# imedslab/OAProgressionMMF

Measured on AMD Instinct MI355X. Metric: knees/sec full XR+MRI+clin fusion train step, higher is better.
Workload: dtype f32; 1 GPU; syn3: XR1MR3C1CnnTrf train step (fwd+FocalLoss+bwd+Adam), per-GPU batch 8, global batch 8, BASELINE config 4 on BASELINE's synthetic tensors: XR 1x310x310 + 3 x MRI 1x160x384x384 (slice-major) + 9 clinical; random-init weights; parallelism=dp1, activation_recompute=012,012,01

## Files before the change

### include/koaf.h

```cpp
#ifndef KOAF_H
#define KOAF_H
#include <stdint.h>
#ifdef __cplusplus
extern "C" {
#endif

#define KOAF_OK 0
#define KOAF_EINVAL (-1)
#define KOAF_ELAUNCH (-2)

int koaf_version(void);
const char* koaf_last_error(void);
int koaf_set_status_buffer(uint32_t* dev4);

typedef struct KoafOperand {
    const float* ptr;
    int64_t ld;
    int64_t bs0, bs1;
    int64_t tap_stride;
    int64_t tap_stride_h;
    int32_t kind;
    int32_t gather;
    int32_t H, W, C;
    int32_t CS;
    int32_t PH, PW;
    int32_t KH, KW, stride, pad;
    int32_t pad_w;
    int32_t _pad1;
    int32_t tf;
    int32_t tf_bs;
    const float* sc;
    const float* sh;
    const uint16_t* planes;
    int64_t plane_stride;
    const float* amax;
    float fscale;
    int32_t _pad4;
    const float* ptr2;
    const float* sc2;
    const uint16_t* zeros;
    float* side;
    const float* sh2;
} KoafOperand;

typedef struct KoafGemm {
    KoafOperand A, B;
    int32_t M, N, K;
    int32_t nb0, nb1;
    int32_t splitk;
    int32_t bm, bn;
    float* C;
    int64_t ldc, cbs0, cbs1;
    float alpha;
    int32_t prec;
    const float* bias;
    const float* residual;
    int64_t ldr, rbs0, rbs1;
    float* stats;
    int64_t stats_ld;
    int64_t stats_bs;
    int32_t cmap, cm_PH, cm_PW, cm_H, cm_W, cm_py, cm_px, _pad2;
    int32_t bnb_mode;
    int32_t fmt;
    const float* bnb_c;
    const float* bnb_y;
    const float* bnb_sc;
    const float* bnb_sh;
    const float* bnb_mean;
    const float* bnb_invstd;
    const float* bnb2_c;
    const float* bnb2_mean;
    const float* bnb2_invstd;
    float* bnb_part;
    float* bnb_amax;
    int32_t m_base, part_row0;
    const float* stats_shift;
    uint32_t* status;
    int32_t act16;
    int32_t _pad5;
    uint16_t* out_planes;
    const float* out_sc;
    const float* out_sh;
    int64_t out_ps;
} KoafGemm;

int koaf_gemm(const KoafGemm* g, void* stream);
int koaf_gemm_pick_tile(const KoafGemm* g, int32_t* bm, int32_t* bn);
int koaf_gemm_part_rows(const KoafGemm* g);
typedef struct KoafLaunchRec {
    char variant[24];
    int32_t bm, bn;
    int32_t tiles, grid_x;
    int32_t splitk, nbatch;
    int32_t fmt, a_tf, b_tf, act16;
    int32_t M, N, K;
    int32_t emit;
} KoafLaunchRec;
int koaf_launch_log(int on);
int koaf_launch_log_read(KoafLaunchRec* out, int32_t cap);
int koaf_slab_reduce(const float* slabs, int32_t nslab, int64_t n, float* out, void* stream);
int koaf_slab_reduce_epilogue(const float* slabs, int32_t nslab, int32_t M, int32_t N, const float* bias,
                              const float* residual, int64_t ldr, float* out, int64_t ldo, void* stream);

typedef struct KoafWPlane {
    int64_t src_off, f_off, d_off, tile0;
    int32_t R, taps, C, Kp, Rp, _pad;
} KoafWPlane;
int koaf_wplanes_build(const float* base, uint16_t* planes, float* amax, const KoafWPlane* table_dev, int32_t n,
                       int64_t ntiles, void* stream);
int koaf_set_conv3x3_halo(int on);
int koaf_set_stream(int on);
int64_t koaf_act_planes_elems(int64_t npix, int32_t C);
int koaf_act_planes(const float* x, const float* x2, int64_t npix, int32_t C, int32_t tf, const float* sc, const float* sh,
                    const float* sc2, const float* amax, float fscale, uint16_t* planes, int32_t act16, void* stream);
typedef struct KoafWImg {
    const uint16_t* f;
    const uint16_t* d;
    const float* amax;
} KoafWImg;
typedef struct KoafBnApply {
    const float* dz;
    const float* c;
    const float* coef;
    const float* amax;
} KoafBnApply;


#define KOAF_ACT_SCALE 16.0f
typedef struct KoafTail {
    const float* idt;
    float* y_out;
    const float* idt_sc;
    const float* idt_sh;
} KoafTail;
typedef struct KoafEmit {
    uint16_t* planes;
    const float* sc;
    const float* sh;
} KoafEmit;
int koaf_conv2d_fwd(const float* x, const float* w, float* y, int32_t N, int32_t H, int32_t W,
                    int32_t Cin, int32_t Cout, int32_t KH, int32_t KW, int32_t stride, int32_t pad,
                    const float* in_sc, const float* in_sh, float* stats, int32_t* stats_rows,
                    const float* stats_shift, const KoafWImg* wimg, const uint16_t* x_planes, const KoafTail* tail,
                    const KoafEmit* emit, int32_t act16, void* stream);
int32_t koaf_conv2d_stats_rows(int64_t M, int32_t Cout);
int koaf_conv2d_dgrad(const float* dy, const float* w, float* dx, int32_t N, int32_t H, int32_t W,
                      int32_t Cin, int32_t Cout, int32_t KH, int32_t KW, int32_t stride,
                      int32_t pad, const float* residual, const KoafWImg* wimg, const float* dy_amax,
                      const KoafBnApply* dy_apply, const uint16_t* dy_planes, int32_t act16, void* stream);
typedef struct KoafBnb {
    int32_t mode, _pad;
    float* dz_amax;
    const float* c;
    const float* y;
    const float* sc;
    const float* sh;
    const float* mean;
    const float* invstd;
    const float* c2;
    const float* mean2;
    const float* invstd2;
} KoafBnb;
int32_t koaf_conv2d_dgrad_bnb_rows(int32_t N, int32_t H, int32_t W, int32_t Cin, int32_t stride);
int koaf_conv2d_dgrad_bnb(const float* dy, const float* w, float* dx, int32_t N, int32_t H, int32_t W,
                          int32_t Cin, int32_t Cout, int32_t KH, int32_t KW, int32_t stride, int32_t pad,
                          const float* residual, const KoafBnb* bnb, float* part, int32_t* part_rows,
                          const KoafWImg* wimg, const float* dy_amax, const KoafBnApply* dy_apply,
                          const uint16_t* dy_planes, int32_t act16, void* stream);
int64_t koaf_conv2d_wgrad_ws(int32_t N, int32_t H, int32_t W, int32_t Cin, int32_t Cout,
                             int32_t KH, int32_t KW, int32_t stride, int32_t pad);
int koaf_conv2d_wgrad(const float* dy, const float* x, float* dw, int32_t N, int32_t H, int32_t W,
                      int32_t Cin, int32_t Cout, int32_t KH, int32_t KW, int32_t stride,
                      int32_t pad, const float* in_sc, const float* in_sh, float* slabs,
                      const float* dy_amax, const KoafBnApply* dy_apply, const uint16_t* dy_planes,
                      const uint16_t* x_planes, int32_t act16, void* stream);

int koaf_gconv_expand_w(const float* w, float* wexp, int32_t C, int32_t groups, float* amax, void* stream);
int koaf_gconv_compress_dw(const float* dwexp, float* dw, int32_t C, int32_t groups, void* stream);
int koaf_gconv3x3_fwd(const float* x, const float* wexp, float* y, int32_t N, int32_t H, int32_t W,
                      int32_t C, int32_t stride, const float* in_sc, const float* in_sh,
                      float* stats, int32_t* stats_rows, const float* stats_shift, const float* w_amax, int32_t act16, void* stream);
int koaf_gconv3x3_dgrad(const float* dy, const float* wexp, float* dx, int32_t N, int32_t H,
                        int32_t W, int32_t C, int32_t stride, const float* w_amax, const float* dy_amax, void* stream);
int64_t koaf_gconv3x3_wgrad_ws(int32_t N, int32_t H, int32_t W, int32_t C, int32_t stride);
int koaf_gconv3x3_wgrad(const float* dy, const float* x, float* dwexp, int32_t N, int32_t H,
                        int32_t W, int32_t C, int32_t stride, const float* in_sc,
                        const float* in_sh, float* slabs, const float* dy_amax, int32_t act16, void* stream);

int32_t koaf_stem_stats_rows(int32_t N, int32_t H);
int koaf_stem_fwd(const float* x, const float* w1t, float* y, int32_t N, int32_t H, int32_t W,
                  float* stats, const float* stats_shift, int32_t act16, void* stream);
int64_t koaf_stem_wgrad_ws(int32_t N, int32_t H, int32_t W);
int koaf_stem_wgrad(const float* dy, const float* x, float* dw1t, int32_t N, int32_t H, int32_t W,
                    float* slabs, const KoafBnApply* dy_apply, int32_t act16, void* stream);
int koaf_stem_fold_w(const float* w, float* w1t, void* stream);
int koaf_stem_unfold_dw(const float* dw1t, float* dw, void* stream);

int koaf_colstats(const float* x, int64_t rows, int32_t C, float* part, int32_t* part_rows,
                  const float* shift, int32_t act16, void* stream);
int32_t koaf_colpart_rows(int64_t rows, int32_t C);
int64_t koaf_bn_reduce_ws(int32_t rows, int32_t C);
int koaf_bn_finalize(const float* stats, int32_t rows, int32_t C, int64_t count,
                     const float* gamma, const float* beta, float* running_mean,
                     float* running_var, int64_t* num_batches_tracked, float momentum, float eps,
                     int32_t train, float* mean, float* invstd, float* sc, float* sh,
                     const float* shift, double* ws, void* stream);
int koaf_bn_add_relu(const float* c, const float* sc, const float* sh, const float* idt,
                     const float* idsc, const float* idsh, float* y, int64_t rows, int32_t C,
                     int32_t act16, void* stream);
int koaf_bn_relu(const float* c, const float* sc, const float* sh, float* y, int64_t rows,
                 int32_t C, int32_t act16, void* stream);
int koaf_bn_bwd_reduce(const float* g, const float* c, const float* ymask, const float* sc,
                       const float* sh, const float* mean, const float* invstd, int32_t mask_mode,
                       float* dz_out, float* part, int32_t* part_rows, int64_t rows, int32_t C,
                       float* dz_amax, int32_t act16, void* stream);
int koaf_bn_bwd_reduce_pool(const float* pool_g, const uint8_t* pool_argmax, const float* c, const float* sc,
                            const float* sh, const float* mean, const float* invstd, float* dz_out, float* part,
                            int32_t* part_rows, int32_t N, int32_t H, int32_t W, int32_t C, float* dz_amax,
                            int32_t act16, void* stream);
int koaf_bn_bwd_finalize(const float* part, int32_t part_rows, int32_t C, int64_t count,
                         const float* sc, const float* invstd, float* dgamma, float* dbeta,
                         float* coef, int32_t nsum, int32_t i1, double* ws, const float* mean,
                         const float* dz_amax, float* amax, void* stream);
int koaf_bn_bwd_apply(const float* dz, const float* c, const float* mean, const float* coef,
                      float* dc, int64_t rows, int32_t C, float* amax, int32_t act16, void* stream);

int koaf_widen(const void* x, int32_t dtype, float* y, int64_t n, void* stream);
int64_t koaf_minmax_ws(int64_t n);
int koaf_minmax(const float* x, int32_t B, int64_t n, float* mm, float* ws, void* stream);
int koaf_augment(const float* x, float* y, const float* mm, const float* params, int32_t B, int32_t R, int32_t C,
                 int32_t S, float mean, float stdv, void* stream);

int koaf_maxpool_fwd(const float* c, const float* sc, const float* sh, float* y, uint8_t* argmax,
                     int32_t N, int32_t H, int32_t W, int32_t C, int32_t act16, void* stream);
int koaf_maxpool_bwd(const float* dy, const uint8_t* argmax, float* da, int32_t N, int32_t H,
                     int32_t W, int32_t C, void* stream);
int koaf_gap_fwd(const float* y, float* out, int32_t N, int32_t HW, int32_t C, int32_t act16, void* stream);
int koaf_gap_bwd(const float* dout, float* dy, int32_t N, int32_t HW, int32_t C, void* stream);

int koaf_slice_fold(const float* x, float* out, int32_t B, int32_t R, int32_t Cc, int32_t S,
                    void* stream);
int koaf_downscale2(const float* x, float* out, int32_t B, int32_t R, int32_t Cc, int32_t S,
                    int32_t fs, void* stream);

int koaf_resize(const float* x, float* out, int64_t BC, int32_t ndim, const int32_t* in_size, const int32_t* out_size,
                void* stream);

int64_t koaf_linear_ws(int32_t M, int32_t N, int32_t K);
int koaf_linear_fwd(const float* x, const float* w, const float* b, const float* residual,
                    float* y, float* ws, int32_t M, int32_t N, int32_t K, void* stream);
int koaf_linear_dgrad(const float* dy, const float* w, const float* residual, float* dx, float* ws,
                      int32_t M, int32_t N, int32_t K, void* stream);
int koaf_linear_wgrad(const float* dy, const float* x, float* dw, float* db, float* ws, int32_t M,
                      int32_t N, int32_t K, void* stream);
int koaf_layernorm_fwd(const float* x, const float* gamma, const float* beta, float* y,
                       float* mean, float* rstd, int32_t rows, int32_t D, float eps, void* stream);
int64_t koaf_layernorm_bwd_ws(int32_t rows, int32_t D);
int koaf_layernorm_bwd(const float* dy, const float* x, const float* gamma, const float* mean,
                       const float* rstd, float* dx, float* dgamma, float* dbeta, float* part,
                       int32_t rows, int32_t D, void* stream);
int koaf_attention_fwd(const float* qkv, float* attn, float* out, int32_t B, int32_t n, int32_t h,
                       int32_t d, float scale, void* stream);
int koaf_attention_bwd(const float* dout, const float* qkv, const float* attn, float* dqkv,
                       float* ws, int32_t B, int32_t n, int32_t h, int32_t d, float scale,
                       void* stream);
int koaf_softmax_rows(float* x, int64_t rows, int32_t n, void* stream);
int koaf_softmax_bwd_rows(float* dp, const float* p, int64_t rows, int32_t n, float scale,
                          void* stream);
int koaf_gelu_fwd(const float* x, float* y, int64_t n, void* stream);
int koaf_gelu_bwd(const float* dy, const float* x, float* dx, int64_t n, void* stream);
int koaf_relu_fwd(const float* x, float* y, int64_t n, void* stream);
int koaf_relu_bwd(const float* dy, const float* y, float* dx, int64_t n, void* stream);
int koaf_dropout(const float* x, float* y, int64_t n, float p, uint64_t seed, const int64_t* epoch, void* stream);
int koaf_counter_add(int64_t* counter, int64_t delta, void* stream);
int koaf_dropout2d(const float* x, float* y, int32_t N, int32_t HW, int32_t C, float p, uint64_t seed,
                   const int64_t* epoch, void* stream);
int koaf_add(const float* a, const float* b, float* out, int64_t n, void* stream);
int64_t koaf_colsum_ws(int32_t rows, int32_t C);
int koaf_colsum(const float* x, float* out, int32_t rows, int32_t C, float* part, void* stream);

int64_t koaf_loss_ws(int32_t B, int64_t S);
int koaf_focal_loss(const float* logits, const int64_t* target, const float* class_weight, float* loss, float* dlogits,
                    int32_t B, int32_t C, int64_t S, float gamma, int32_t reduction_mean, float* ws, void* stream);
int koaf_ce_loss(const float* logits, const int64_t* target, const float* class_weight, float* loss, float* dlogits,
                 int32_t B, int32_t C, int64_t S, float* ws, void* stream);

int koaf_adam_step(float* p, const float* g, float* m, float* v, int64_t n, float lr, double beta1,
                   double beta2, float eps, float weight_decay, int32_t step, int32_t adamw,
                   const float* hyper, float* vmax, void* stream);
int koaf_adam_hyper(int32_t* step, const float* lr, double beta1, double beta2, float* hyper, void* stream);
int koaf_fill(float* p, float value, int64_t n, void* stream);

#ifdef __cplusplus
}
#endif
#endif
```

### oaprogressionmmf_amd/_lib.py

```python
import ctypes
import os
import re
from pathlib import Path

_ROOT = Path(__file__).resolve().parent
HEADER = _ROOT.parent / "include" / "koaf.h"
LIB_PATH = _ROOT / "csrc" / "libkoaf.so"


class KoafOperand(ctypes.Structure):
    _fields_ = [
        ("ptr", ctypes.c_void_p),
        ("ld", ctypes.c_int64),
        ("bs0", ctypes.c_int64),
        ("bs1", ctypes.c_int64),
        ("tap_stride", ctypes.c_int64),
        ("tap_stride_h", ctypes.c_int64),
        ("kind", ctypes.c_int32),
        ("gather", ctypes.c_int32),
        ("H", ctypes.c_int32),
        ("W", ctypes.c_int32),
        ("C", ctypes.c_int32),
        ("CS", ctypes.c_int32),
        ("PH", ctypes.c_int32),
        ("PW", ctypes.c_int32),
        ("KH", ctypes.c_int32),
        ("KW", ctypes.c_int32),
        ("stride", ctypes.c_int32),
        ("pad", ctypes.c_int32),
        ("pad_w", ctypes.c_int32),
        ("_pad1", ctypes.c_int32),
        ("tf", ctypes.c_int32),
        ("tf_bs", ctypes.c_int32),
        ("sc", ctypes.c_void_p),
        ("sh", ctypes.c_void_p),
        ("planes", ctypes.c_void_p),
        ("plane_stride", ctypes.c_int64),
        ("amax", ctypes.c_void_p),
        ("fscale", ctypes.c_float),
        ("_pad4", ctypes.c_int32),
        ("ptr2", ctypes.c_void_p),
        ("sc2", ctypes.c_void_p),
        ("zeros", ctypes.c_void_p),
        ("side", ctypes.c_void_p),
        ("sh2", ctypes.c_void_p),
    ]


class KoafGemm(ctypes.Structure):
    _fields_ = [
        ("A", KoafOperand),
        ("B", KoafOperand),
        ("M", ctypes.c_int32),
        ("N", ctypes.c_int32),
        ("K", ctypes.c_int32),
        ("nb0", ctypes.c_int32),
        ("nb1", ctypes.c_int32),
        ("splitk", ctypes.c_int32),
        ("bm", ctypes.c_int32),
        ("bn", ctypes.c_int32),
        ("C", ctypes.c_void_p),
        ("ldc", ctypes.c_int64),
        ("cbs0", ctypes.c_int64),
        ("cbs1", ctypes.c_int64),
        ("alpha", ctypes.c_float),
        ("prec", ctypes.c_int32),
        ("bias", ctypes.c_void_p),
        ("residual", ctypes.c_void_p),
        ("ldr", ctypes.c_int64),
        ("rbs0", ctypes.c_int64),
        ("rbs1", ctypes.c_int64),
        ("stats", ctypes.c_void_p),
        ("stats_ld", ctypes.c_int64),
        ("stats_bs", ctypes.c_int64),
        ("cmap", ctypes.c_int32),
        ("cm_PH", ctypes.c_int32),
        ("cm_PW", ctypes.c_int32),
        ("cm_H", ctypes.c_int32),
        ("cm_W", ctypes.c_int32),
        ("cm_py", ctypes.c_int32),
        ("cm_px", ctypes.c_int32),
        ("_pad2", ctypes.c_int32),
        ("bnb_mode", ctypes.c_int32),
        ("fmt", ctypes.c_int32),
        ("bnb_c", ctypes.c_void_p),
        ("bnb_y", ctypes.c_void_p),
        ("bnb_sc", ctypes.c_void_p),
        ("bnb_sh", ctypes.c_void_p),
        ("bnb_mean", ctypes.c_void_p),
        ("bnb_invstd", ctypes.c_void_p),
        ("bnb2_c", ctypes.c_void_p),
        ("bnb2_mean", ctypes.c_void_p),
        ("bnb2_invstd", ctypes.c_void_p),
        ("bnb_part", ctypes.c_void_p),
        ("bnb_amax", ctypes.c_void_p),
        ("m_base", ctypes.c_int32),
        ("part_row0", ctypes.c_int32),
        ("stats_shift", ctypes.c_void_p),
        ("status", ctypes.c_void_p),
        ("act16", ctypes.c_int32),
        ("_pad5", ctypes.c_int32),
        ("out_planes", ctypes.c_void_p),
        ("out_sc", ctypes.c_void_p),
        ("out_sh", ctypes.c_void_p),
        ("out_ps", ctypes.c_int64),
    ]


class KoafBnb(ctypes.Structure):
    _fields_ = [
        ("mode", ctypes.c_int32),
        ("_pad", ctypes.c_int32),
        ("dz_amax", ctypes.c_void_p),
        ("c", ctypes.c_void_p),
        ("y", ctypes.c_void_p),
        ("sc", ctypes.c_void_p),
        ("sh", ctypes.c_void_p),
        ("mean", ctypes.c_void_p),
        ("invstd", ctypes.c_void_p),
        ("c2", ctypes.c_void_p),
        ("mean2", ctypes.c_void_p),
        ("invstd2", ctypes.c_void_p),
    ]


class KoafWPlane(ctypes.Structure):
    _fields_ = [
        ("src_off", ctypes.c_int64),
        ("f_off", ctypes.c_int64),
        ("d_off", ctypes.c_int64),
        ("tile0", ctypes.c_int64),
        ("R", ctypes.c_int32),
        ("taps", ctypes.c_int32),
        ("C", ctypes.c_int32),
        ("Kp", ctypes.c_int32),
        ("Rp", ctypes.c_int32),
        ("_pad", ctypes.c_int32),
    ]


class KoafWImg(ctypes.Structure):
    _fields_ = [("f", ctypes.c_void_p), ("d", ctypes.c_void_p), ("amax", ctypes.c_void_p)]


class KoafTail(ctypes.Structure):
    _fields_ = [("idt", ctypes.c_void_p), ("y_out", ctypes.c_void_p), ("idt_sc", ctypes.c_void_p), ("idt_sh", ctypes.c_void_p)]


class KoafEmit(ctypes.Structure):
    _fields_ = [("planes", ctypes.c_void_p), ("sc", ctypes.c_void_p), ("sh", ctypes.c_void_p)]


class KoafBnApply(ctypes.Structure):
    _fields_ = [("dz", ctypes.c_void_p), ("c", ctypes.c_void_p), ("coef", ctypes.c_void_p), ("amax", ctypes.c_void_p)]


class KoafLaunchRec(ctypes.Structure):
    _fields_ = [
        ("variant", ctypes.c_char * 24),
        ("bm", ctypes.c_int32),
        ("bn", ctypes.c_int32),
        ("tiles", ctypes.c_int32),
        ("grid_x", ctypes.c_int32),
        ("splitk", ctypes.c_int32),
        ("nbatch", ctypes.c_int32),
        ("fmt", ctypes.c_int32),
        ("a_tf", ctypes.c_int32),
        ("b_tf", ctypes.c_int32),
        ("act16", ctypes.c_int32),
        ("M", ctypes.c_int32),
        ("N", ctypes.c_int32),
        ("K", ctypes.c_int32),
        ("emit", ctypes.c_int32),
    ]


_SCALARS = {
    "int": ctypes.c_int,
    "int32_t": ctypes.c_int32,
    "int64_t": ctypes.c_int64,
    "uint64_t": ctypes.c_uint64,
    "uint32_t": ctypes.c_uint32,
    "float": ctypes.c_float,
    "double": ctypes.c_double,
}


def _ctype(decl: str):
    decl = decl.strip()
    if "*" in decl:
        base = decl.replace("const", "").replace("*", "").split()[0]
        if base == "KoafGemm":
            return ctypes.POINTER(KoafGemm)
        if base == "KoafBnb":
            return ctypes.POINTER(KoafBnb)
        if base == "KoafWImg":
            return ctypes.POINTER(KoafWImg)
        if base == "KoafBnApply":
            return ctypes.POINTER(KoafBnApply)
        if base == "KoafTail":
            return ctypes.POINTER(KoafTail)
        if base == "KoafEmit":
            return ctypes.POINTER(KoafEmit)
        if base == "KoafLaunchRec":
            return ctypes.POINTER(KoafLaunchRec)
        if base == "char":
            return ctypes.c_char_p
        return ctypes.c_void_p
    toks = decl.replace("const", "").split()
    return _SCALARS[toks[0]]


def parse_header(path=HEADER):
    text = Path(path).read_text()
    text = re.sub(r"/\*.*?\*/", " ", text, flags=re.S)
    text = re.sub(r"typedef struct.*?\}\s*\w+;", " ", text, flags=re.S)
    text = re.sub(r"^\s*#.*$", " ", text, flags=re.M)
    protos = {}
    for m in re.finditer(r"([\w\s\*]+?)\b(koaf_\w+)\s*\(([^)]*)\)\s*;", text):
        ret, name, args = m.group(1).strip(), m.group(2), m.group(3).strip()
        if args in ("void", ""):
            argtypes = []
        else:
            argtypes = []
            for a in args.split(","):
                a = a.strip()
                mm = re.match(r"(.*?)(\w+)$", a)
                argtypes.append(_ctype(mm.group(1) if mm.group(1).strip() else a))
        protos[name] = (_ctype(ret) if ret != "void" else None, argtypes)
    return protos


_LIB = None


class KoafError(RuntimeError):
    pass


def lib():
    global _LIB
    if _LIB is not None:
        return _LIB
    path = Path(os.environ.get("KOAF_LIB", LIB_PATH))
    if not path.exists():
        raise KoafError(
            f"libkoaf.so not found at {path}: build it with `python -c 'import __graft_entry__ as g; "
            f"g.build()'` or `make -C oaprogressionmmf_amd/csrc` -- there is no CPU fallback")
    handle = ctypes.CDLL(str(path))
    for name, (restype, argtypes) in parse_header().items():
        fn = getattr(handle, name)
        fn.restype = restype
        fn.argtypes = argtypes
    _LIB = handle
    return _LIB


def check(rc, what=""):
    if rc != 0:
        msg = lib().koaf_last_error()
        raise KoafError(f"{what}: rc={rc}: {msg.decode() if msg else '?'}")
```

### oaprogressionmmf_amd/csrc/koaf_common.h

```cpp
#pragma once
#include <hip/hip_runtime.h>
#include <stdint.h>
#include <stdio.h>
#include "../../include/koaf.h"

typedef float v4f __attribute__((ext_vector_type(4)));
typedef float v16f __attribute__((ext_vector_type(16)));
typedef int v4i __attribute__((ext_vector_type(4)));
typedef long long v4l __attribute__((ext_vector_type(4)));

void koaf_set_error(const char* fmt, ...);

#define KOAF_REQUIRE(cond, ...)            \
    do {                                   \
        if (!(cond)) {                     \
            koaf_set_error(__VA_ARGS__);   \
            return KOAF_EINVAL;            \
        }                                  \
    } while (0)

static inline int koaf_check_launch(const char* what) {
    hipError_t e = hipGetLastError();
    if (e != hipSuccess) {
        koaf_set_error("%s: launch failed: %s", what, hipGetErrorString(e));
        return KOAF_ELAUNCH;
    }
    return KOAF_OK;
}

static inline int64_t cdiv64(int64_t a, int64_t b) { return (a + b - 1) / b; }
static inline bool aligned16(const void* p) { return (((uintptr_t)p) & 15) == 0; }

__device__ __forceinline__ float wave_sum(float v) {
#pragma unroll
    for (int o = 32; o > 0; o >>= 1) v += __shfl_xor(v, o, 64);
    return v;
}
__device__ __forceinline__ float wave_max(float v) {
#pragma unroll
    for (int o = 32; o > 0; o >>= 1) v = fmaxf(v, __shfl_xor(v, o, 64));
    return v;
}

__device__ __forceinline__ unsigned koaf_absbits(float x) { return __float_as_uint(x) & 0x7fffffffu; }
__device__ __forceinline__ bool koaf_bits_finite(unsigned absbits) { return absbits < 0x7f800000u; }
__device__ __forceinline__ unsigned wave_max_u(unsigned v) {
#pragma unroll
    for (int o = 32; o > 0; o >>= 1) { const unsigned w = (unsigned)__shfl_xor((int)v, o, 64); v = v > w ? v : w; }
    return v;
}

__device__ __forceinline__ void block_amax_raise_bits(unsigned bits, float* slot) {
    __shared__ unsigned koaf_amax_red[16];
    bits = wave_max_u(bits);
    const int w = threadIdx.x >> 6, nw = (blockDim.x + 63) >> 6;
    if ((threadIdx.x & 63) == 0) koaf_amax_red[w] = bits;
    __syncthreads();
    if (threadIdx.x == 0) {
        unsigned m = koaf_amax_red[0];
        for (int i = 1; i < nw; ++i) m = m > koaf_amax_red[i] ? m : koaf_amax_red[i];
        if (m > __hip_atomic_load(reinterpret_cast<unsigned*>(slot), __ATOMIC_RELAXED, __HIP_MEMORY_SCOPE_AGENT))
            atomicMax(reinterpret_cast<unsigned*>(slot), m);
    }
}
__device__ __forceinline__ void block_amax_raise(float v, float* slot) { block_amax_raise_bits(koaf_absbits(v), slot); }

uint32_t* koaf_status_ptr();
__device__ __forceinline__ void koaf_status_add(uint32_t* st, int slot, unsigned n) {
    if (st != nullptr && n != 0u) atomicAdd(&st[slot], n);
}

typedef __bf16 koaf_bf16x2 __attribute__((ext_vector_type(2)));
__device__ __forceinline__ v4f widen_bf16x4(unsigned lo, unsigned hi) {
    return (v4f){__uint_as_float(lo << 16), __uint_as_float(lo & 0xffff0000u), __uint_as_float(hi << 16), __uint_as_float(hi & 0xffff0000u)};
}
__device__ __forceinline__ uint2 round_bf16x4(v4f v) {
    typedef float v2f_ __attribute__((ext_vector_type(2)));
    const unsigned a = __builtin_bit_cast(unsigned, __builtin_convertvector((v2f_){v[0], v[1]}, koaf_bf16x2));
    const unsigned b = __builtin_bit_cast(unsigned, __builtin_convertvector((v2f_){v[2], v[3]}, koaf_bf16x2));
    return make_uint2(a, b);
}
template <bool H>
__device__ __forceinline__ v4f load4_nt(const float* p, int64_t off) {
    if constexpr (!H) return __builtin_nontemporal_load((const v4f*)(p + off));
    else {
        const unsigned short* q = reinterpret_cast<const unsigned short*>(p) + off;
        const unsigned lo = __builtin_nontemporal_load((const unsigned*)q), hi = __builtin_nontemporal_load((const unsigned*)q + 1);
        return widen_bf16x4(lo, hi);
    }
}
template <bool H>
__device__ __forceinline__ void store4_nt(float* p, int64_t off, v4f v) {
    if constexpr (!H) __builtin_nontemporal_store(v, (v4f*)(p + off));
    else {
        const uint2 u = round_bf16x4(v);
        unsigned* q = (unsigned*)(reinterpret_cast<unsigned short*>(p) + off);
        __builtin_nontemporal_store(u.x, q);
        __builtin_nontemporal_store(u.y, q + 1);
    }
}

template <bool H>
__device__ __forceinline__ v4f load4(const float* p, int64_t off) {
    if constexpr (!H) return *(const v4f*)(p + off);
    else {
        const uint2 u = *(const uint2*)(reinterpret_cast<const unsigned short*>(p) + off);
        return widen_bf16x4(u.x, u.y);
    }
}
template <bool H>
__device__ __forceinline__ void store4(float* p, int64_t off, v4f v) {
    if constexpr (!H) *(v4f*)(p + off) = v;
    else *(uint2*)(reinterpret_cast<unsigned short*>(p) + off) = round_bf16x4(v);
}
```

### oaprogressionmmf_amd/csrc/koaf_conv.hip

```cpp
#include <string.h>
#include "koaf_common.h"
#include <stdlib.h>

namespace {

inline void zero_gemm(KoafGemm* g) { *g = KoafGemm{}; g->alpha = 1.f; g->nb0 = g->nb1 = 1; g->splitk = 1; }

inline int conv_out(int H, int K, int s, int p) { return (H + 2 * p - K) / s + 1; }

inline int64_t rup32(int64_t v) { return (v + 31) / 32 * 32; }

inline void set_fimg(KoafGemm* g, const KoafWImg* w, int R, int64_t K) {
    g->fmt = 1;
    g->A.fscale = KOAF_ACT_SCALE;
    g->B.amax = w->amax;
    if (!w->f) return;
    g->B.kind = 2; g->B.gather = 0;
    g->B.planes = w->f; g->B.ld = rup32(K); g->B.plane_stride = (int64_t)R * g->B.ld;
}

inline void set_aplanes(KoafOperand* a, const uint16_t* planes, int64_t plane_elems) {
    a->kind = 2; a->planes = planes; a->plane_stride = plane_elems; a->zeros = planes + 2 * plane_elems;
    a->ptr = nullptr; a->ptr2 = nullptr; a->tf = 0; a->sc = a->sh = a->sc2 = nullptr;
}
// ... 95 lines not shown
            if (oy < OH) {
                if (ox < OW) put((((int64_t)n * OH + oy) * OW + ox) * 64 + co, a0);
                if (ox + 1 < OW) put((((int64_t)n * OH + oy) * OW + ox + 1) * 64 + co, a1);
            }
        }
    }
    if constexpr (ST) {
        __shared__ float sred[2][ST_TH][64];
        sred[0][pg][co] = s1;
        sred[1][pg][co] = s2;
        __syncthreads();
        if (pg < 2) {
            float a = 0.f;
#pragma unroll
            for (int g = 0; g < ST_TH; ++g) a += sred[pg][g][co];
            part[((int64_t)blockIdx.x * 2 + pg) * 64 + co] = a;
        }
    }
}

template <bool APPLY, bool C16>
__global__ void __launch_bounds__(256) stem_wgrad_kernel(const float* __restrict__ dy, const float* __restrict__ x,
                                                         float* __restrict__ slabs, int N, int H, int W, int OH,
                                                         int OW, const float* __restrict__ cc, const float* __restrict__ coef) {
    __shared__ __attribute__((aligned(16))) float patch[ST_PH][ST_PW];
    __shared__ float red[3][64][49 + 1];
    const int co = threadIdx.x & 63, pg = threadIdx.x >> 6;
    const int tx = (OW + ST_TW - 1) / ST_TW, ty = (OH + ST_TH - 1) / ST_TH;
    const int ntile = N * ty * tx;
    float acc[49];
#pragma unroll
    for (int k = 0; k < 49; ++k) acc[k] = 0.f;
    float k0 = 1.f, k2 = 0.f, k3 = 0.f;
    if constexpr (APPLY) { k0 = coef[co]; k2 = coef[128 + co]; k3 = coef[192 + co]; }
    auto grad = [&](int64_t o) {
        float gv = dy[o];
        if constexpr (APPLY) {
            float cv;
            if constexpr (C16) cv = __uint_as_float((unsigned)reinterpret_cast<const unsigned short*>(cc)[o] << 16);
            else cv = cc[o];
            gv = fmaf(k0, gv, fmaf(-k2, cv, k3));
        }
        return gv;
    };
    for (int tile = blockIdx.x; tile < ntile; tile += gridDim.x) {
        int b = tile;
        const int bx = b % tx; b /= tx;
        const int by = b % ty;
        const int n = b / ty;
        const int oy0 = by * ST_TH, ox0 = bx * ST_TW;
        __syncthreads();
        stem_load_patch(patch, x, n, H, W, oy0, ox0);
        __syncthreads();
        const int oy = oy0 + pg;
#pragma unroll 1
        for (int q = 0; q < ST_TW / 2; ++q) {
            const int ox = ox0 + 2 * q;
            float g0 = 0.f, g1 = 0.f;
            if (oy < OH) {
                if (ox < OW) g0 = grad((((int64_t)n * OH + oy) * OW + ox) * 64 + co);
                if (ox + 1 < OW) g1 = grad((((int64_t)n * OH + oy) * OW + ox + 1) * 64 + co);
            }
#pragma unroll
            for (int kh = 0; kh < 7; ++kh) {
                const float* pr = &patch[2 * pg + kh][4 * q];
                const v4f p0 = *(const v4f*)pr, p1 = *(const v4f*)(pr + 4);
                const float p8 = pr[8];
                const float pv[9] = {p0[0], p0[1], p0[2], p0[3], p1[0], p1[1], p1[2], p1[3], p8};
#pragma unroll
                for (int kw = 0; kw < 7; ++kw) acc[kh * 7 + kw] += g0 * pv[kw] + g1 * pv[kw + 2];
            }
        }
    }
    __syncthreads();
    if (pg > 0) {
#pragma unroll
        for (int k = 0; k < 49; ++k) red[pg - 1][co][k] = acc[k];
    }
    __syncthreads();
    if (pg == 0) {
        float* sl = slabs + (int64_t)blockIdx.x * 49 * 64;
#pragma unroll
        for (int k = 0; k < 49; ++k) sl[k * 64 + co] = acc[k] + red[0][co][k] + red[1][co][k] + red[2][co][k];
    }
}

__global__ void stem_fold_kernel(const float* __restrict__ w, float* __restrict__ w1t) {
    const int i = blockIdx.x * blockDim.x + threadIdx.x;
    if (i >= 64 * 49) return;
    const int co = i / 49, k = i - co * 49;
    const float* s = w + (int64_t)i * 3;
    w1t[k * 64 + co] = s[0] + s[1] + s[2];
}
__global__ void stem_unfold_kernel(const float* __restrict__ dw1t, float* __restrict__ dw) {
    const int i = blockIdx.x * blockDim.x + threadIdx.x;
    if (i >= 64 * 49) return;
    const int co = i / 49, k = i - co * 49;
    const float v = dw1t[k * 64 + co];
    dw[(int64_t)i * 3 + 0] = v;
    dw[(int64_t)i * 3 + 1] = v;
    dw[(int64_t)i * 3 + 2] = v;
}

__global__ void __launch_bounds__(256) gconv_expand_kernel(const float* __restrict__ w, float* __restrict__ wexp,
                                                           int C, int Cg, float* __restrict__ amax) {
    const int64_t total = (int64_t)C * 9 * 64;
    unsigned mb = 0u;
    for (int64_t i = (int64_t)blockIdx.x * 256 + threadIdx.x; i < total; i += (int64_t)gridDim.x * 256) {
        const int ci = (int)(i & 63);
        int64_t r = i >> 6;
        const int tap = (int)(r % 9);
        const int co = (int)(r / 9);
        const int col = co & 63;
        const int g0 = (col / Cg) * Cg;
        float v = 0.f;
        if (ci >= g0 && ci < g0 + Cg) v = w[((int64_t)co * 9 + tap) * Cg + (ci - g0)];
        wexp[i] = v;
        mb = max(mb, koaf_absbits(v));
    }
    if (amax != nullptr) block_amax_raise_bits(mb, amax);
}
__global__ void __launch_bounds__(256) gconv_compress_kernel(const float* __restrict__ dwexp, float* __restrict__ dw,
                                                             int C, int Cg) {
    const int64_t total = (int64_t)C * 9 * Cg;
    for (int64_t i = (int64_t)blockIdx.x * 256 + threadIdx.x; i < total; i += (int64_t)gridDim.x * 256) {
        const int cg = (int)(i % Cg);
        int64_t r = i / Cg;
        const int tap = (int)(r % 9);
        const int co = (int)(r / 9);
        const int g0 = ((co & 63) / Cg) * Cg;
        dw[i] = dwexp[((int64_t)co * 9 + tap) * 64 + g0 + cg];
    }
}

}

#define STREAM ((hipStream_t)stream)

extern "C" int koaf_conv2d_fwd(const float* x, const float* w, float* y, int32_t N, int32_t H, int32_t W, int32_t Cin,
                               int32_t Cout, int32_t KH, int32_t KW, int32_t stride, int32_t pad, const float* in_sc,
                               const float* in_sh, float* stats, int32_t* stats_rows, const float* stats_shift,
                               const KoafWImg* wimg, const uint16_t* x_planes, const KoafTail* tail, const KoafEmit* emit,
                               int32_t act16, void* stream) {
    KOAF_REQUIRE((x || x_planes) && w && y && N > 0 && Cin % 32 == 0 && Cout % 4 == 0, "koaf_conv2d_fwd: bad args (Cin=%d Cout=%d)",
                 Cin, Cout);
    KOAF_REQUIRE(!tail || (tail->idt && x && in_sc && in_sh && !x_planes && KH == 1 && KW == 1 && stride == 1 && pad == 0 && wimg &&
                           wimg->amax && wimg->f && (tail->idt_sc == nullptr) == (tail->idt_sh == nullptr)),
                 "koaf_conv2d_fwd: the fused bottleneck tail serves 1x1 / stride-1 convolutions with weight plane images, from x / in_sc / in_sh");
    KOAF_REQUIRE((in_sc == nullptr) == (in_sh == nullptr), "koaf_conv2d_fwd: in_sc/in_sh come together");
    const int OH = conv_out(H, KH, stride, pad), OW = conv_out(W, KW, stride, pad);
    const int64_t M = (int64_t)N * OH * OW;
    KOAF_REQUIRE(M < (1ll << 31), "koaf_conv2d_fwd: too many output pixels");
    KoafGemm g;
    zero_gemm(&g);
    g.A.ptr = x;
    g.A.kind = 0;
    if (KH == 1 && KW == 1 && stride == 1 && pad == 0 && !x_planes) {
        g.A.gather = 0;
        g.A.ld = Cin;
    } else {
        g.A.gather = 1;
        g.A.H = H; g.A.W = W; g.A.C = Cin; g.A.CS = Cin;
        g.A.PH = OH; g.A.PW = OW;
        g.A.KH = KH; g.A.KW = KW; g.A.stride = stride; g.A.pad = pad; g.A.pad_w = pad;
    }
    if (in_sc) { g.A.tf = 1; g.A.sc = in_sc; g.A.sh = in_sh; }
    if (tail) { g.A.tf = 3; g.A.ptr2 = tail->idt; g.A.side = tail->y_out; g.A.sc2 = tail->idt_sc; g.A.sh2 = tail->idt_sc ? tail->idt_sh : nullptr; }
    g.B.ptr = w;
    g.B.kind = 0;
    g.B.ld = (int64_t)KH * KW * Cin;
    g.M = (int)M; g.N = Cout; g.K = KH * KW * Cin;
    if (wimg && wimg->amax) set_fimg(&g, wimg, Cout, g.K);
    if (x_planes) {
        KOAF_REQUIRE(g.A.gather == 1 && g.B.kind == 2, "koaf_conv2d_fwd: x_planes serve the gathered kernels and need wimg->f");
        set_aplanes(&g.A, x_planes, (int64_t)N * H * W * Cin);
    }
    g.C = y; g.ldc = Cout;
    g.stats = stats;
    g.stats_shift = stats ? stats_shift : nullptr;
    g.act16 = act16 ? 1 : 0;
    if (emit) {
        KOAF_REQUIRE(emit->planes && emit->sc && emit->sh && (Cout % 8) == 0, "koaf_conv2d_fwd: emit needs planes / sc / sh and Cout %% 8 == 0");
        g.out_planes = emit->planes; g.out_sc = emit->sc; g.out_sh = emit->sh; g.out_ps = M * Cout;
    }
    if (stats_rows) *stats_rows = koaf_gemm_part_rows(&g);
    return koaf_gemm(&g, stream);
}

extern "C" int32_t koaf_conv2d_stats_rows(int64_t M, int32_t Cout) { return (int32_t)cdiv64(M, 64); }

static void set_apply(KoafOperand* a, const KoafBnApply* ap, int C) {
    a->ptr = ap->dz; a->ptr2 = ap->c; a->tf = 2;
    a->sc = ap->coef; a->sc2 = ap->coef + 2 * (int64_t)C; a->sh = ap->coef + 3 * (int64_t)C;
    a->amax = ap->amax;
}

static void set_bnb(KoafGemm* g, const KoafBnb* b, float* part) {
    if (!b) return;
    g->bnb_amax = b->dz_amax;
    g->bnb_mode = b->mode;
    g->bnb_c = b->c; g->bnb_y = b->y; g->bnb_sc = b->sc; g->bnb_sh = b->sh;
    g->bnb_mean = b->mean; g->bnb_invstd = b->invstd;
    g->bnb2_c = b->c2; g->bnb2_mean = b->mean2; g->bnb2_invstd = b->invstd2;
    g->bnb_part = part;
}

extern "C" int32_t koaf_conv2d_dgrad_bnb_rows(int32_t N, int32_t H, int32_t W, int32_t Cin, int32_t stride) {
    if (stride == 2) {
        int64_t r = 0;
        for (int py = 0; py < 2; ++py)
            for (int px = 0; px < 2; ++px) r += cdiv64((int64_t)N * ((H - py + 1) / 2) * ((W - px + 1) / 2), 64);
        return (int32_t)r;
    }
    return (int32_t)cdiv64((int64_t)N * H * W, 64);
}

extern "C" int koaf_conv2d_dgrad_bnb(const float* dy, const float* w, float* dx, int32_t N, int32_t H, int32_t W,
                                     int32_t Cin, int32_t Cout, int32_t KH, int32_t KW, int32_t stride, int32_t pad,
                                     const float* residual, const KoafBnb* bnb, float* part, int32_t* part_rows,
                                     const KoafWImg* wimg, const float* dy_amax, const KoafBnApply* dy_apply,
                                     const uint16_t* dy_planes, int32_t act16, void* stream) {
    KOAF_REQUIRE(!dy_planes || (wimg && wimg->amax && wimg->d && (dy_amax || dy_apply) && KH * KW > 1),
                 "koaf_conv2d_dgrad: dy_planes need the weight's D plane image, dy_amax and a gathered (KH*KW > 1) kernel");
    KOAF_REQUIRE((dy || dy_apply || dy_planes) && w && dx && N > 0 && Cout % 32 == 0 && Cin % 4 == 0, "koaf_conv2d_dgrad: bad args");
    KOAF_REQUIRE(!dy_apply || (dy_apply->dz && dy_apply->c && dy_apply->coef && dy_apply->amax && wimg && wimg->amax && wimg->d),
                 "koaf_conv2d_dgrad: dy_apply needs dz / c / coef / amax and the weight's D plane image");
    if (dy_apply) { dy = dy_apply->dz; dy_amax = dy_apply->amax; }
    if (bnb && bnb->dz_amax && hipMemsetAsync(bnb->dz_amax, 0, sizeof(float), (hipStream_t)stream) != hipSuccess) {
        koaf_set_error("koaf_conv2d_dgrad_bnb: memset failed");
        return KOAF_ELAUNCH;
    }
    const bool f16 = wimg && wimg->amax && dy_amax;
    const bool ps = f16 && wimg->d != nullptr;
    const uint16_t* w_dimg = ps ? wimg->d : nullptr;
    const int64_t dld = (int64_t)KH * KW * Cout, dps = (int64_t)Cin * dld;
    KOAF_REQUIRE(!bnb || (part && part_rows), "koaf_conv2d_dgrad_bnb: part / part_rows required");
    const int nsum = (bnb && bnb->c2) ? 3 : 2;
    int rows_done = 0;
    const int OH = conv_out(H, KH, stride, pad), OW = conv_out(W, KW, stride, pad);
    const int64_t M = (int64_t)N * H * W;
    KOAF_REQUIRE(M < (1ll << 31), "koaf_conv2d_dgrad: too many pixels");
    KoafGemm g;
    if (stride == 2) {
        for (int py = 0; py < 2; ++py)
            for (int px = 0; px < 2; ++px) {
                const int Hc = (H - py + 1) / 2, Wc = (W - px + 1) / 2;
                if (Hc <= 0 || Wc <= 0) continue;
                const int khs = (py + pad) & 1, kws = (px + pad) & 1;
                const int nkh = khs < KH ? (KH - khs + 1) / 2 : 0, nkw = kws < KW ? (KW - kws + 1) / 2 : 0;
                const int offy = (py + pad - khs) / 2, offx = (px + pad - kws) / 2;
                zero_gemm(&g);
                g.prec = 1;
                if (f16) { g.fmt = 1; g.A.amax = dy_amax; g.B.amax = wimg->amax; }
                g.A.ptr = dy; g.A.kind = 0; g.A.gather = 2;
                if (dy_apply) set_apply(&g.A, dy_apply, Cout);
                g.A.H = OH; g.A.W = OW; g.A.C = Cout; g.A.CS = Cout;
                g.A.PH = Hc; g.A.PW = Wc;
                g.A.KH = nkh > 0 ? nkh : 1; g.A.KW = nkw > 0 ? nkw : 1; g.A.stride = 1; g.A.pad = offy; g.A.pad_w = offx;
                g.B.ptr = w + ((int64_t)khs * KW + kws) * Cin; g.B.kind = 1; g.B.gather = 3;
                g.B.C = Cout; g.B.ld = (int64_t)KH * KW * Cin;
                g.B.KW = g.A.KW; g.B.tap_stride = 2ll * Cin; g.B.tap_stride_h = 2ll * KW * Cin;
                if (ps) {
                    g.B.kind = 2; g.B.gather = 0;
                    g.B.planes = w_dimg + ((int64_t)khs * KW + kws) * Cout; g.B.ld = dld; g.B.plane_stride = dps;
                    g.B.tap_stride = 2ll * Cout; g.B.tap_stride_h = 2ll * KW * Cout;
                }
                if (dy_planes && nkh > 0 && nkw > 0) set_aplanes(&g.A, dy_planes, (int64_t)N * OH * OW * Cout);
                g.M = N * Hc * Wc; g.N = Cin; g.K = nkh * nkw * Cout;
                g.C = dx; g.ldc = Cin;
                g.residual = residual; g.ldr = Cin;
                g.cmap = 1; g.cm_PH = Hc; g.cm_PW = Wc; g.cm_H = H; g.cm_W = W; g.cm_py = py; g.cm_px = px;
                if (bnb) {
                    set_bnb(&g, bnb, part + (int64_t)rows_done * nsum * Cin);
                    rows_done += koaf_gemm_part_rows(&g);
                }
                g.act16 = act16 ? 2 : 0;
                int rc = koaf_gemm(&g, stream);
                if (rc != KOAF_OK) return rc;
            }
        if (part_rows) *part_rows = rows_done;
        return KOAF_OK;
    }
    zero_gemm(&g);
    g.prec = 1;
    if (f16) { g.fmt = 1; g.A.amax = dy_amax; g.B.amax = wimg->amax; }
    g.A.ptr = dy;
    g.A.kind = 0;
    if (dy_apply) set_apply(&g.A, dy_apply, Cout);
    g.B.ptr = w;
    g.B.kind = 1;
    if (KH == 1 && KW == 1 && stride == 1 && pad == 0) {
        g.A.gather = 0;
        g.A.ld = Cout;
        g.B.gather = 0;
        g.B.ld = Cin;
    } else {
        g.A.gather = 2;
        g.A.H = OH; g.A.W = OW; g.A.C = Cout; g.A.CS = Cout;
        g.A.PH = H; g.A.PW = W;
        g.A.KH = KH; g.A.KW = KW; g.A.stride = stride; g.A.pad = pad; g.A.pad_w = pad;
        g.B.gather = 3;
        g.B.C = Cout;
        g.B.ld = (int64_t)KH * KW * Cin;
        g.B.KW = KW;
        g.B.tap_stride = Cin;
        g.B.tap_stride_h = (int64_t)KW * Cin;
    }
    if (ps) {
        g.B.kind = 2; g.B.gather = 0; g.B.C = 0; g.B.tap_stride = g.B.tap_stride_h = 0;
        g.B.planes = w_dimg; g.B.ld = dld; g.B.plane_stride = dps;
    }
    if (dy_planes) set_aplanes(&g.A, dy_planes, (int64_t)N * OH * OW * Cout);
    g.M = (int)M; g.N = Cin; g.K = KH * KW * Cout;
    g.C = dx; g.ldc = Cin;
    g.residual = residual; g.ldr = Cin;
    if (bnb) {
        set_bnb(&g, bnb, part);
        *part_rows = koaf_gemm_part_rows(&g);
    }
    g.act16 = act16 ? 2 : 0;
    return koaf_gemm(&g, stream);
}

extern "C" int koaf_conv2d_dgrad(const float* dy, const float* w, float* dx, int32_t N, int32_t H, int32_t W,
                                 int32_t Cin, int32_t Cout, int32_t KH, int32_t KW, int32_t stride, int32_t pad,
                                 const float* residual, const KoafWImg* wimg, const float* dy_amax,
                                 const KoafBnApply* dy_apply, const uint16_t* dy_planes, int32_t act16, void* stream) {
    return koaf_conv2d_dgrad_bnb(dy, w, dx, N, H, W, Cin, Cout, KH, KW, stride, pad, residual, nullptr, nullptr,
                                 nullptr, wimg, dy_amax, dy_apply, dy_planes, act16, stream);
}

bool koaf_wgrad3_ring_ok(int N, int H, int W, int Cin, int Cout);
int64_t koaf_wgrad3_ring_ws(int N, int H, int W, int Cin, int Cout);
int koaf_wgrad3_ring(const uint16_t* dy_planes, const uint16_t* x_planes, float* dw, float* slabs, const float* dy_amax,
                     float x_scale, int N, int H, int W, int Cin, int Cout, void* stream);
static inline bool wgrad3_ring_shape(int N, int H, int W, int Cin, int Cout, int KH, int KW, int stride, int pad) {
    return KH == 3 && KW == 3 && stride == 1 && pad == 1 && koaf_wgrad3_ring_ok(N, H, W, Cin, Cout);
}

extern "C" int64_t koaf_conv2d_wgrad_ws(int32_t N, int32_t H, int32_t W, int32_t Cin, int32_t Cout, int32_t KH,
                                        int32_t KW, int32_t stride, int32_t pad) {
    const int OH = conv_out(H, KH, stride, pad), OW = conv_out(W, KW, stride, pad);
    WgradPlan p = wgrad_plan(Cout, KH * KW * Cin, (int64_t)N * OH * OW, Cin, 1);
    int64_t ws = p.splitk > 1 ? (int64_t)(p.splitk + 16) * Cout * KH * KW * Cin : 0;
    if (wgrad3_ring_shape(N, H, W, Cin, Cout, KH, KW, stride, pad)) {
        const int64_t w3 = koaf_wgrad3_ring_ws(N, H, W, Cin, Cout);
        if (w3 > ws) ws = w3;
    }
    return ws;
}

extern "C" int koaf_conv2d_wgrad(const float* dy, const float* x, float* dw, int32_t N, int32_t H, int32_t W,
                                 int32_t Cin, int32_t Cout, int32_t KH, int32_t KW, int32_t stride, int32_t pad,
                                 const float* in_sc, const float* in_sh, float* slabs, const float* dy_amax,
                                 const KoafBnApply* dy_apply, const uint16_t* dy_planes, const uint16_t* x_planes,
                                 int32_t act16, void* stream) {
    KOAF_REQUIRE((dy_planes == nullptr) == (x_planes == nullptr) && (!dy_planes || dy_amax || dy_apply),
                 "koaf_conv2d_wgrad: dy_planes and x_planes come together, with dy_amax (or dy_apply)");
    KOAF_REQUIRE((dy || dy_apply || dy_planes) && (x || x_planes) && dw && N > 0 && Cin % 64 == 0 && Cout % 4 == 0, "koaf_conv2d_wgrad: bad args");
    KOAF_REQUIRE(!dy_apply || (dy_apply->dz && dy_apply->c && dy_apply->coef && dy_apply->amax),
                 "koaf_conv2d_wgrad: dy_apply needs dz / c / coef / amax");
    if (dy_apply) { dy = dy_apply->dz; dy_amax = dy_apply->amax; }
    KOAF_REQUIRE((in_sc == nullptr) == (in_sh == nullptr), "koaf_conv2d_wgrad: in_sc/in_sh come together");
    const int OH = conv_out(H, KH, stride, pad), OW = conv_out(W, KW, stride, pad);
    const int64_t P = (int64_t)N * OH * OW;
    KOAF_REQUIRE(P < (1ll << 31), "koaf_conv2d_wgrad: too many pixels");
    const int Ntot = KH * KW * Cin;
    if (dy_planes && slabs && wgrad3_ring_shape(N, H, W, Cin, Cout, KH, KW, stride, pad))
        return koaf_wgrad3_ring(dy_planes, x_planes, dw, slabs, dy_amax, KOAF_ACT_SCALE, N, H, W, Cin, Cout, stream);
    WgradPlan p = wgrad_plan(Cout, Ntot, P, Cin, 1);
    KOAF_REQUIRE(p.splitk == 1 || slabs, "koaf_conv2d_wgrad: workspace required");
    KoafGemm g;
    zero_gemm(&g);
    g.prec = 1;
    if (dy_amax) { g.fmt = 1; g.A.amax = dy_amax; g.B.fscale = KOAF_ACT_SCALE; }
    g.A.ptr = dy; g.A.kind = 1; g.A.ld = Cout;
    if (dy_apply) set_apply(&g.A, dy_apply, Cout);
    g.B.ptr = x; g.B.kind = 1;
    if (KH == 1 && KW == 1 && stride == 1 && pad == 0) {
        g.B.gather = 0;
        g.B.ld = Cin;
    } else {
        g.B.gather = 1;
        g.B.H = H; g.B.W = W; g.B.C = Cin; g.B.CS = Cin;
        g.B.PH = OH; g.B.PW = OW;
        g.B.KH = KH; g.B.KW = KW; g.B.stride = stride; g.B.pad = pad; g.B.pad_w = pad;
    }
    if (in_sc) { g.B.tf = 1; g.B.sc = in_sc; g.B.sh = in_sh; }
    if (dy_planes) {
        set_aplanes(&g.A, dy_planes, P * Cout);
        g.A.kind = 3; g.A.ld = Cout;
        set_aplanes(&g.B, x_planes, (int64_t)N * H * W * Cin);
        g.B.kind = 3; g.B.gather = 1;
        g.B.H = H; g.B.W = W; g.B.C = Cin; g.B.CS = Cin;
        g.B.PH = OH; g.B.PW = OW;
        g.B.KH = KH; g.B.KW = KW; g.B.stride = stride; g.B.pad = pad; g.B.pad_w = pad;
    }
    g.M = Cout; g.N = Ntot; g.K = (int)P;
    g.bm = p.bm; g.bn = p.bn; g.splitk = p.splitk;
    g.C = p.splitk > 1 ? slabs : dw;
    g.ldc = Ntot;
    g.act16 = (act16 && !dy_planes) ? 3 : 0;
    int rc = koaf_gemm(&g, stream);
    if (rc != KOAF_OK || p.splitk == 1) return rc;
    return koaf_slab_reduce(slabs, p.splitk, (int64_t)Cout * Ntot, dw, stream);
}

extern "C" int koaf_gconv_expand_w(const float* w, float* wexp, int32_t C, int32_t groups, float* amax, void* stream) {
    KOAF_REQUIRE(w && wexp && C % 64 == 0 && groups > 0 && C % groups == 0 && 64 % (C / groups) == 0,
                 "koaf_gconv_expand_w: C=%d groups=%d unsupported", C, groups);
    hipLaunchKernelGGL(gconv_expand_kernel, dim3(1024), dim3(256), 0, STREAM, w, wexp, C, C / groups, amax);
    return koaf_check_launch("koaf_gconv_expand_w");
}
extern "C" int koaf_gconv_compress_dw(const float* dwexp, float* dw, int32_t C, int32_t groups, void* stream) {
    KOAF_REQUIRE(dwexp && dw && C % 64 == 0 && groups > 0 && C % groups == 0 && 64 % (C / groups) == 0,
                 "koaf_gconv_compress_dw: C=%d groups=%d unsupported", C, groups);
    hipLaunchKernelGGL(gconv_compress_kernel, dim3(512), dim3(256), 0, STREAM, dwexp, dw, C, C / groups);
    return koaf_check_launch("koaf_gconv_compress_dw");
}

extern "C" int koaf_gconv3x3_fwd(const float* x, const float* wexp, float* y, int32_t N, int32_t H, int32_t W,
                                 int32_t C, int32_t stride, const float* in_sc, const float* in_sh, float* stats,
                                 int32_t* stats_rows, const float* stats_shift, const float* w_amax, int32_t act16, void* stream) {
    KOAF_REQUIRE(x && wexp && y && N > 0 && C % 64 == 0, "koaf_gconv3x3_fwd: bad args");
    const int OH = conv_out(H, 3, stride, 1), OW = conv_out(W, 3, stride, 1);
    const int64_t M = (int64_t)N * OH * OW;
    KOAF_REQUIRE(M < (1ll << 31), "koaf_gconv3x3_fwd: too many pixels");
    KoafGemm g;
    zero_gemm(&g);
    g.nb1 = C / 64;
    g.A.ptr = x; g.A.kind = 0; g.A.gather = 1; g.A.bs1 = 64;
    g.A.H = H; g.A.W = W; g.A.C = 64; g.A.CS = C; g.A.PH = OH; g.A.PW = OW;
    g.A.KH = 3; g.A.KW = 3; g.A.stride = stride; g.A.pad = 1; g.A.pad_w = 1;
    if (in_sc) { g.A.tf = 1; g.A.sc = in_sc; g.A.sh = in_sh; }
    g.B.ptr = wexp; g.B.kind = 0; g.B.ld = 576; g.B.bs1 = 64 * 576;
    g.M = (int)M; g.N = 64; g.K = 576;
    g.C = y; g.ldc = C; g.cbs1 = 64;
    g.stats = stats; g.stats_ld = C; g.stats_bs = 64;
    g.stats_shift = stats ? stats_shift : nullptr;
    g.bn = 64; g.bm = 128;
    if (stats_rows) *stats_rows = (int)cdiv64(M, g.bm);
    g.A.tf_bs = 64;
    g.act16 = act16 ? 1 : 0;
    if (w_amax && !act16) { g.fmt = 1; g.A.fscale = KOAF_ACT_SCALE; g.B.amax = w_amax; }
    return koaf_gemm(&g, stream);
}

extern "C" int koaf_gconv3x3_dgrad(const float* dy, const float* wexp, float* dx, int32_t N, int32_t H, int32_t W,
                                   int32_t C, int32_t stride, const float* w_amax, const float* dy_amax, void* stream) {
    KOAF_REQUIRE(dy && wexp && dx && N > 0 && C % 64 == 0, "koaf_gconv3x3_dgrad: bad args");
    const int OH = conv_out(H, 3, stride, 1), OW = conv_out(W, 3, stride, 1);
    const int64_t M = (int64_t)N * H * W;
    KOAF_REQUIRE(M < (1ll << 31), "koaf_gconv3x3_dgrad: too many pixels");
    KoafGemm g;
    zero_gemm(&g);
    g.prec = 1;
    g.nb1 = C / 64;
    g.A.ptr = dy; g.A.kind = 0; g.A.gather = 2; g.A.bs1 = 64;
    g.A.H = OH; g.A.W = OW; g.A.C = 64; g.A.CS = C; g.A.PH = H; g.A.PW = W;
    g.A.KH = 3; g.A.KW = 3; g.A.stride = stride; g.A.pad = 1; g.A.pad_w = 1;
    g.B.ptr = wexp; g.B.kind = 1; g.B.gather = 3; g.B.C = 64; g.B.ld = 576; g.B.tap_stride = 64;
    g.B.tap_stride_h = 3 * 64; g.B.KW = 3;
    g.B.bs1 = 64 * 576;
    g.M = (int)M; g.N = 64; g.K = 576;
    g.C = dx; g.ldc = C; g.cbs1 = 64;
    g.bn = 64; g.bm = 128;
    if (w_amax && dy_amax) { g.fmt = 1; g.A.amax = dy_amax; g.B.amax = w_amax; }
    return koaf_gemm(&g, stream);
}

extern "C" int64_t koaf_gconv3x3_wgrad_ws(int32_t N, int32_t H, int32_t W, int32_t C, int32_t stride) {
    const int OH = conv_out(H, 3, stride, 1), OW = conv_out(W, 3, stride, 1);
    WgradPlan p = wgrad_plan(64, 576, (int64_t)N * OH * OW, 64, C / 64);
    return (int64_t)p.splitk * C * 576;
}

extern "C" int koaf_gconv3x3_wgrad(const float* dy, const float* x, float* dwexp, int32_t N, int32_t H, int32_t W,
                                   int32_t C, int32_t stride, const float* in_sc, const float* in_sh, float* slabs,
                                   const float* dy_amax, int32_t act16, void* stream) {
    KOAF_REQUIRE(dy && x && dwexp && slabs && N > 0 && C % 64 == 0, "koaf_gconv3x3_wgrad: bad args");
    const int OH = conv_out(H, 3, stride, 1), OW = conv_out(W, 3, stride, 1);
    const int64_t P = (int64_t)N * OH * OW;
// ... 304 lines not shown
```

### oaprogressionmmf_amd/csrc/koaf_elem.hip

```cpp
#include <stdarg.h>
#include "koaf_common.h"
#include <stdlib.h>

static thread_local char g_err[512] = "";
void koaf_set_error(const char* fmt, ...) {
    va_list ap;
    va_start(ap, fmt);
    vsnprintf(g_err, sizeof(g_err), fmt, ap);
    va_end(ap);
}
extern "C" const char* koaf_last_error(void) { return g_err; }
static uint32_t* g_status = nullptr;
uint32_t* koaf_status_ptr() { return g_status; }
extern "C" int koaf_set_status_buffer(uint32_t* dev4) { g_status = dev4; return KOAF_OK; }
extern "C" int koaf_version(void) { return 190; }

namespace {

constexpr int EB = 256;

inline int ew_blocks_per_cu() {
    static const int v = [] { const char* e = getenv("KOAF_EW_BLOCKS_PER_CU"); int n = e ? atoi(e) : 32; return n < 1 ? 1 : n; }();
    return v;
}
inline unsigned ew_grid(int64_t nvec) {
    int64_t b = cdiv64(nvec, EB);
    if (b > 256 * ew_blocks_per_cu()) b = 256 * ew_blocks_per_cu();
    if (b < 1) b = 1;
    return (unsigned)b;
}

struct ColGeom {
    int CW;
    int nchunk;
    int CV;
    int RP;
    int rpb;
    int nblk;
};
inline bool col_geom(int64_t rows, int C, int max_blk, ColGeom* g) {
    if (C % 4) return false;
    int CW = C > 1024 ? 1024 : C;
    if (C % CW) return false;
    int CV = CW / 4;
    if (256 % CV) return false;
    g->CW = CW;
    g->nchunk = C / CW;
    g->CV = CV;
    g->RP = 256 / CV;
    int64_t rpb = cdiv64(rows, max_blk);
    rpb = cdiv64(rpb, g->RP) * g->RP;
    if (rpb < g->RP * 4) rpb = g->RP * 4;
    g->rpb = (int)rpb;
    g->nblk = (int)cdiv64(rows, rpb);
    return true;
}

template <int NS>
__device__ __forceinline__ void col_block_reduce(v4f (&s)[NS], float* part, int blk, int C, int c0, int CV,
                                                 int RP) {
    __shared__ v4f red[256];
    const int t = threadIdx.x;
    const int cvx = t % CV, ry = t / CV;
#pragma unroll
    for (int k = 0; k < NS; ++k) {
        __syncthreads();
        red[t] = s[k];
        __syncthreads();
        if (ry == 0) {
            v4f a = red[cvx];
            for (int j = 1; j < RP; ++j) a += red[j * CV + cvx];
            *(v4f*)&part[((int64_t)blk * NS + k) * C + c0 + 4 * cvx] = a;
        }
    }
}

template <bool H>
__global__ void __launch_bounds__(256) colstats_kernel(const float* __restrict__ x, int64_t rows, int C,
                                                       ColGeom g, float* __restrict__ part, int sq,
                                                       const float* __restrict__ shift) {
    const int t = threadIdx.x, cvx = t % g.CV, ry = t / g.CV;
    const int c0 = blockIdx.y * g.CW;
    const int64_t rbeg = (int64_t)blockIdx.x * g.rpb;
    const int64_t rend = min(rows, rbeg + (int64_t)g.rpb);
    v4f s[2] = {{0, 0, 0, 0}, {0, 0, 0, 0}};
    v4f k = {0, 0, 0, 0};
    if (shift) k = *(const v4f*)&shift[c0 + 4 * cvx];
    for (int64_t r = rbeg + ry; r < rend; r += g.RP) {
        v4f v = load4<H>(x, r * C + c0 + 4 * cvx) - k;
        s[0] += v;
        s[1] += v * v;
    }
    if (sq) col_block_reduce<2>(s, part, blockIdx.x, C, c0, g.CV, g.RP);
    else {
        v4f s1[1] = {s[0]};
        col_block_reduce<1>(s1, part, blockIdx.x, C, c0, g.CV, g.RP);
    }
}

__global__ void colsum_small_kernel(const float* __restrict__ x, int rows, int C, float* __restrict__ out) {
    int c = blockIdx.x * blockDim.x + threadIdx.x;
    if (c >= C) return;
    float a = 0.f;
    for (int r = 0; r < rows; ++r) a += x[(int64_t)r * C + c];
    out[c] = a;
}

template <int NS>
__global__ void __launch_bounds__(1024) colfinal_kernel(const float* __restrict__ part, int rows, int C,
                                                        float* __restrict__ out0, float* __restrict__ out1) {
    __shared__ double red[NS][16][64];
    const int cx = threadIdx.x & 63, gy = threadIdx.x >> 6;
    const int c = blockIdx.x * 64 + cx;
    double a[NS];
#pragma unroll
    for (int k = 0; k < NS; ++k) a[k] = 0.0;
    if (c < C)
        for (int r = gy; r < rows; r += 16)
#pragma unroll
            for (int k = 0; k < NS; ++k) a[k] += (double)part[((int64_t)r * NS + k) * C + c];
#pragma unroll
    for (int k = 0; k < NS; ++k) red[k][gy][cx] = a[k];
    __syncthreads();
    if (gy == 0 && c < C) {
#pragma unroll
        for (int k = 0; k < NS; ++k) {
            double s = 0.0;
            for (int j = 0; j < 16; ++j) s += red[k][j][cx];
            (k == 0 ? out0 : out1)[c] = (float)s;
        }
    }
}

__global__ void __launch_bounds__(1024) part_reduce_kernel(const float* __restrict__ src, int rows, int C, int nsum,
                                                           int i1, int chunk, double* __restrict__ ws) {
    __shared__ double red[2][16][64];
    const int cx = threadIdx.x & 63, gy = threadIdx.x >> 6;
    const int c = blockIdx.x * 64 + cx;
    const int r0 = blockIdx.y * chunk, r1 = min(rows, r0 + chunk);
    double a = 0.0, b = 0.0;
    if (c < C)
        for (int r = r0 + gy; r < r1; r += 16) {
            a += (double)src[((int64_t)r * nsum + 0) * C + c];
            b += (double)src[((int64_t)r * nsum + i1) * C + c];
        }
    red[0][gy][cx] = a;
    red[1][gy][cx] = b;
    __syncthreads();
    if (gy < 2 && c < C) {
        double t = 0.0;
        for (int j = 0; j < 16; ++j) t += red[gy][j][cx];
        ws[((int64_t)blockIdx.y * 2 + gy) * C + c] = t;
    }
}

static inline int part_slices(int rows) { return rows > 128 ? (rows >= 4096 ? 64 : (rows + 63) / 64) : 0; }

template <typename T>
__global__ void __launch_bounds__(1024) bn_finalize_kernel(const T* __restrict__ stats, int rows, int C,
                                                           double inv_count, double unbias,
                                                           const float* __restrict__ gamma,
                                                           const float* __restrict__ beta, float* running_mean,
                                                           float* running_var, int64_t* nbt, float momentum,
                                                           float eps, int train, float* mean, float* invstd,
                                                           float* sc, float* sh, const float* __restrict__ shift,
                                                           uint32_t* status) {
    __shared__ double red[2][16][64];
    const int cx = threadIdx.x & 63, gy = threadIdx.x >> 6;
// ... 1283 lines not shown
```

### oaprogressionmmf_amd/csrc/koaf_gemm.hip

```cpp
#include "koaf_gemm_launch.h"
#include <stdlib.h>
#include <string.h>
#include <atomic>
#include <mutex>
#include <vector>

namespace {

__global__ void __launch_bounds__(256) slab_reduce_epi_kernel(const float* __restrict__ slabs, int nslab, int M, int N,
                                                              const float* __restrict__ bias,
                                                              const float* __restrict__ residual, int64_t ldr,
                                                              float* __restrict__ out, int64_t ldo) {
    const int N4 = N / 4;
    const int64_t total = (int64_t)M * N4;
    const int64_t n = (int64_t)M * N;
    for (int64_t i = (int64_t)blockIdx.x * 256 + threadIdx.x; i < total; i += (int64_t)gridDim.x * 256) {
        const int m = (int)(i / N4), c = (int)(i - (int64_t)m * N4) * 4;
        v4f a = *(const v4f*)(slabs + (int64_t)m * N + c);
        for (int s = 1; s < nslab; ++s) a += *(const v4f*)(slabs + (int64_t)s * n + (int64_t)m * N + c);
        if (bias) a += *(const v4f*)(bias + c);
        if (residual) a += *(const v4f*)(residual + (int64_t)m * ldr + c);
        *(v4f*)(out + (int64_t)m * ldo + c) = a;
    }
}

__global__ void __launch_bounds__(256) slab_reduce_kernel(const float* __restrict__ slabs, int nslab,
                                                          int64_t n, float* __restrict__ out) {
    __shared__ v4f red[4][64];
    const int cx = threadIdx.x & 63, gy = threadIdx.x >> 6;
    const int64_t i = ((int64_t)blockIdx.x * 64 + cx) * 4;
    const int s_per = (nslab + gridDim.y - 1) / gridDim.y;
    const int s0 = blockIdx.y * s_per, s1 = min(nslab, s0 + s_per);
    v4f a = {0.f, 0.f, 0.f, 0.f};
    if (i < n)
        for (int s = s0 + gy; s < s1; s += 4) a += *(const v4f*)(slabs + (int64_t)s * n + i);
    red[gy][cx] = a;
    __syncthreads();
    if (gy == 0 && i < n) {
        a = red[0][cx] + red[1][cx] + red[2][cx] + red[3][cx];
        if (gridDim.y == 1) *(v4f*)(out + i) = a;
        else *(v4f*)(out + (int64_t)blockIdx.y * n + i) = a;
    }
}

bool operand_vec_ok(const KoafOperand& o, int R, int K) {
    if (o.kind == 3) {
        return aligned16(o.planes) && aligned16(o.zeros) && o.zeros && !(o.plane_stride & 7) && !(o.bs0 & 7) && !(o.bs1 & 7) &&
               !(R & 7) && (o.gather ? (o.C > 0 && !(o.C & 7) && !(o.CS & 7) && o.KW > 0) : !(o.ld & 7));
    }
    if (o.kind == 2 && o.gather) {
        return aligned16(o.planes) && aligned16(o.zeros) && o.zeros && !(o.plane_stride & 7) && !(o.bs0 & 7) && !(o.bs1 & 7) &&
               o.C > 0 && !(o.C & 31) && !(o.CS & 7) && o.KW > 0 && (K % BK) == 0;
    }
    if (o.kind == 2) {
        if (!aligned16(o.planes) || (o.ld & 7) || (o.plane_stride & 7) || (o.bs0 & 7) || (o.bs1 & 7)) return false;
        if ((o.tap_stride & 7) || (o.tap_stride_h & 7) || o.C <= 0 || (o.C & 31) || o.KW <= 0) return false;
        return true;
    }
    if (!aligned16(o.ptr)) return false;
    if ((o.ld & 3) || (o.bs0 & 3) || (o.bs1 & 3)) return false;
    if (o.kind == 0) {
        if (K & 3) return false;
        if (o.gather && ((o.C & 31) || (o.CS & 3))) return false;
    } else {
        if (R & 3) return false;
        if (o.gather == 3 && ((o.C & 31) || (o.tap_stride & 3) || (o.tap_stride_h & 3))) return false;
        if (o.gather == 1 && ((o.C & 3) || (o.CS & 3))) return false;
    }
    if (o.tf && (!aligned16(o.sc) || !aligned16(o.sh))) return false;
    if (o.tf == 2 && (!aligned16(o.sc2) || !aligned16(o.ptr2))) return false;
    return true;
}

}

namespace {
std::atomic<int> g_log_on{0};
std::mutex g_log_mutex;
std::vector<KoafLaunchRec> g_log;
int64_t g_log_seen = 0;
constexpr size_t LOG_CAP = 4096;

}

void koaf_log_launch(const char* variant, const KoafGemm& g, dim3 grid, dim3 launched) {
    if (!g_log_on.load(std::memory_order_relaxed)) return;
    KoafLaunchRec r;
    memset(&r, 0, sizeof(r));
    strncpy(r.variant, variant, sizeof(r.variant) - 1);
    r.bm = g.bm; r.bn = g.bn;
    r.tiles = (int32_t)grid.x; r.grid_x = (int32_t)launched.x;
    r.splitk = (int32_t)launched.y; r.nbatch = (int32_t)launched.z;
    r.fmt = g.fmt; r.a_tf = g.A.tf; r.b_tf = g.B.tf; r.act16 = g.act16;
    r.M = g.M - g.m_base; r.N = g.N; r.K = g.K;
    r.emit = g.out_planes != nullptr;
    std::lock_guard<std::mutex> lock(g_log_mutex);
    ++g_log_seen;
    if (g_log.size() < LOG_CAP) g_log.push_back(r);
}

namespace {
int g_stream_mode = -1;
bool stream_ok(const KoafGemm& g) {
    if (g_stream_mode < 0) { const char* e = getenv("KOAF_STREAM"); g_stream_mode = (e && e[0] == '0') ? 0 : 1; }
    return g_stream_mode == 1 && g.A.kind == 0 && g.A.gather == 0 && g.K >= 2 * BK && (g.K % (2 * BK)) == 0 && g.splitk == 1 &&
           g.nb0 * g.nb1 == 1 && (g.A.tf != 1 || g.K <= STREAM_TAB_K);
}
}

extern "C" int koaf_gemm_pick_tile(const KoafGemm* g, int32_t* bm, int32_t* bn) {
    int b_m = g->bm, b_n = g->bn;
    const int64_t batch = (int64_t)g->nb0 * g->nb1 * (g->splitk > 0 ? g->splitk : 1);
    if (b_n == 0) {
        b_n = (g->N >= 128) ? 128 : 64;
        if (g->B.kind == 1 && g->B.gather == 1 && (g->B.C % 64) != 0) b_n = 64;
    }
    if (b_m == 0) b_m = (g->M >= 128) ? 128 : 64;
    if (g->bm == 0 || g->bn == 0) {
        auto tiles = [&](int m, int n) { return cdiv64(g->M, m) * cdiv64(g->N, n) * batch; };
        constexpr int64_t fill = 384;
        if (g->bm == 0 && tiles(b_m, b_n) < fill && b_m == 128) b_m = 64;
        if (g->bn == 0 && tiles(b_m, b_n) < fill && b_n == 128) b_n = 64;
    }
    *bm = b_m;
    *bn = b_n;
    return KOAF_OK;
}

namespace {
int g_halo_mode = 1;
int g_t2d_mode = -1;

bool halo_ok(const KoafGemm& g) {
    const KoafOperand& a = g.A;
    return g_halo_mode != 0 && a.kind == 2 && (a.gather == 1 || a.gather == 2) && a.KH == 3 && a.KW == 3 && a.stride == 1 && a.pad == 1 &&
           a.pad_w == 1 && a.PH == a.H && a.PW == a.W && a.W <= halo_max_w(g.N >= 128 ? 128 : 64, 256) && a.H * a.W > 0 && (g.M % (a.H * a.W)) == 0 &&
           g.nb0 * g.nb1 == 1 && g.m_base == 0 && g.K == 9 * a.C && g.B.kind == 2 && g.fmt == 1 && !g.cmap && g.splitk == 1;
}

bool gemm_vec_ok(const KoafGemm& g) {
    bool vec = operand_vec_ok(g.A, g.M, g.K) && operand_vec_ok(g.B, g.N, g.K);
    if ((g.N & 3) || !aligned16(g.C) || (g.ldc & 3) || (g.cbs0 & 3) || (g.cbs1 & 3)) vec = false;
    if (g.residual && (!aligned16(g.residual) || (g.ldr & 3) || (g.rbs0 & 3) || (g.rbs1 & 3))) vec = false;
    if (g.bias && !aligned16(g.bias)) vec = false;
    return vec;
}

TilePlan plan_tiles(const KoafGemm& g) {
    TilePlan t;
    KoafGemm q = g;
    koaf_gemm_pick_tile(&q, &t.bm, &t.bn);
    t.vec = gemm_vec_ok(g);
    if (!t.vec) { t.bm = 64; t.bn = 64; }
    t.halo = t.vec && halo_ok(g);
    if (g_t2d_mode < 0) { const char* e = getenv("KOAF_CONV3_T2D"); g_t2d_mode = (e && e[0] == '0') ? 0 : ((e && e[0] == '2') ? 2 : 1); }
    t.t2d = t.halo && g_t2d_mode >= 1 && g_halo_mode == 1 && (g.A.C == 64 || (g.A.C == 128 && g_t2d_mode == 2)) && (g.N == 64 || g.N == 128) &&
            (g.A.W % 16) == 0 && (g.A.H % 8) == 0 && g.A.zeros != nullptr;
    if (t.t2d) {
        t.halo = false;
        t.bm = 128;
        t.bn = 64;
    } else if (t.halo) {
        t.bn = g.N >= 128 ? 128 : 64;
        const bool fits128 = g.A.W <= halo_max_w(t.bn, 128);
        t.bm = (g_halo_mode == 3 || (g_halo_mode == 1 && g.A.C <= 64)) && fits128 ? 128 : 256;
    }
    t.part_rows = (int)cdiv64(g.M - g.m_base, t.bm);
    t.stream = t.vec && g.fmt == 1 && g.act16 == 0 && t.bm == 128 && operand_mode(g.A) == M_KC && operand_mode(g.B) == M_PS && !g.B.tf &&
               !(g.out_planes && g.A.tf == 2) && stream_ok(g);
    return t;
}
}

static void fill_defaults(KoafGemm& g) {
    if (g.nb0 < 1) g.nb0 = 1;
    if (g.nb1 < 1) g.nb1 = 1;
    if (g.splitk < 1) g.splitk = 1;
    if (g.A.CS == 0) g.A.CS = g.A.C;
    if (g.B.CS == 0) g.B.CS = g.B.C;
    if (g.stats_ld == 0) g.stats_ld = g.N;
    if (g.B.kind == 2 && g.B.C == 0) { g.B.C = ((g.K + BK - 1) / BK) * BK; g.B.KW = 1; }
}

namespace {
int launch_wplanes(const KoafGemm& g, const TilePlan& tp, dim3 grid, hipStream_t s) {
    switch (g.act16) {
        case 0: return koaf_launch_wplanes_act0(g, tp, grid, s);
        case 1: return koaf_launch_wplanes_act1(g, tp, grid, s);
        case 2: return koaf_launch_wplanes_act2(g, tp, grid, s);
    }
    return KOAF_NO_KERNEL;
}

int launch_planned(const KoafGemm& g, const TilePlan& tp, dim3 grid, hipStream_t s) {
    const int am = operand_mode(g.A), bm = operand_mode(g.B);
    if (g.out_planes && (tp.t2d || tp.halo)) { koaf_set_error("koaf_gemm: out_planes is not built for the 3x3 plane-image kernels"); return KOAF_EINVAL; }
    if ((tp.t2d || tp.halo) && g.act16 == 3) {
        koaf_set_error(tp.t2d ? "koaf_gemm: 2-D tile kernel with act16 = 3" : "koaf_gemm: halo kernel with act16 = 3");
        return KOAF_EINVAL;
    }
    if (tp.t2d || tp.halo) return launch_wplanes(g, tp, grid, s);
    if (g.fmt == 1) KOAF_REQUIRE(tp.vec, "koaf_gemm: the fp16 scheme needs the vector path (16-B aligned operands, K %% 4 == 0, N %% 4 == 0)");
    else if (!tp.vec && g.act16 != 0) { koaf_set_error("koaf_gemm: bf16 activation storage needs the vector path"); return KOAF_EINVAL; }
    int rc = KOAF_NO_KERNEL;
    if (tp.stream) rc = koaf_launch_stream(g, tp, grid, s);
    else if (g.out_planes) {
        if (g.fmt == 1 && am == M_KC && bm == M_PS) rc = launch_wplanes(g, tp, grid, s);
        if (rc == KOAF_NO_KERNEL) {
            koaf_set_error("koaf_gemm: out_planes is built for dense K-contiguous A x weight plane images on the fp16 scheme (1x1 forward convolutions); "
                           "got operand modes (%d,%d) tf=%d fmt=%d act16=%d", am, bm, g.A.tf, (int)(g.fmt == 1), g.act16);
            return KOAF_EINVAL;
        }
    }
    else if (bm == M_PS) rc = launch_wplanes(g, tp, grid, s);
    else if (am == M_PK) rc = koaf_launch_kmajor(g, tp, grid, s);
    else rc = g.fmt == 1 ? koaf_launch_fp16(g, tp, grid, s) : koaf_launch_bf16(g, tp, grid, s);
    if (rc == KOAF_NO_KERNEL) {
        koaf_set_error("koaf_gemm: operand mode pair (%d,%d) tf=(%d,%d) fmt=%d vec=%d act16=%d is not instantiated", am, bm, g.A.tf, g.B.tf,
                       (int)(g.fmt == 1), (int)tp.vec, g.act16);
        return KOAF_EINVAL;
    }
    return rc;
}
}

extern "C" int koaf_gemm_part_rows(const KoafGemm* gp) {
    KoafGemm g = *gp;
    fill_defaults(g);
    return plan_tiles(g).part_rows;
}

extern "C" int koaf_gemm(const KoafGemm* gp, void* stream) {
    KoafGemm g = *gp;
    KOAF_REQUIRE(g.M > 0 && g.N > 0 && g.K >= 0, "koaf_gemm: bad dims M=%d N=%d K=%d", g.M, g.N, g.K);
    KOAF_REQUIRE((g.A.kind >= 2 ? (const void*)g.A.planes : (const void*)g.A.ptr) &&
                 (g.B.kind >= 2 ? (const void*)g.B.planes : (const void*)g.B.ptr) && g.C, "koaf_gemm: null operand");
    fill_defaults(g);
    if (!g.status) g.status = koaf_status_ptr();
    KOAF_REQUIRE(!g.cmap || (g.splitk == 1 && !g.stats), "koaf_gemm: row map excludes split-K / stats");
    KOAF_REQUIRE(!g.bnb_mode || (g.splitk == 1 && !g.stats && g.nb0 * g.nb1 == 1 && g.bnb_c && g.bnb_mean &&
                                 g.bnb_invstd && g.bnb_part && (g.bnb_mode == 1 ? g.bnb_y != nullptr
                                                                                 : (g.bnb_sc && g.bnb_sh))),
                 "koaf_gemm: fused BN-backward epilogue needs c/mean/invstd/part (+y or sc/sh), no split-K/batch");
    KOAF_REQUIRE(g.splitk == 1 || (!g.bias && !g.residual && !g.stats),
                 "koaf_gemm: split-K writes raw slabs (no epilogue)");
    KOAF_REQUIRE((int64_t)g.nb0 * g.nb1 <= 65535 && g.splitk <= 65535, "koaf_gemm: batch/splitk too large");
    KOAF_REQUIRE(g.A.kind == 0 || (g.A.kind == 1 && g.A.gather == 0) || g.A.kind == 2 || (g.A.kind == 3 && g.A.gather == 0),
                 "koaf_gemm: A is K-contiguous fp32, K-major without gather, or activation plane images");
    KOAF_REQUIRE((g.A.kind == 3) == (g.B.kind == 3), "koaf_gemm: K-major plane images (kind 3) come as a pair");
    if (g.A.kind == 3)
        KOAF_REQUIRE(g.fmt == 1 && !g.A.tf && !g.B.tf && g.A.zeros && g.B.zeros && (g.B.gather == 0 || g.B.gather == 1),
                     "koaf_gemm: K-major plane images need fmt 1, no transform, the zero chunks; B.gather 0 | 1");
    if (g.A.kind == 2)
        KOAF_REQUIRE((g.A.gather == 1 || g.A.gather == 2) && g.B.kind == 2 && g.fmt == 1 && !g.A.tf && g.splitk == 1 && g.A.zeros,
                     "koaf_gemm: activation plane images (A.kind 2) need gather 1|2, a pre-split B, fmt 1, no transform, no split-K");
    KOAF_REQUIRE(!(g.A.kind == 0 && g.A.gather == 3) && !(g.B.kind == 0 && g.B.gather == 3),
                 "koaf_gemm: tapped gather needs a K-major operand");
    KOAF_REQUIRE(!(g.B.kind == 0 && g.B.gather), "koaf_gemm: K-contiguous B cannot be gathered");
    KOAF_REQUIRE(g.fmt == 0 || g.fmt == 1, "koaf_gemm: fmt must be 0 (bf16 x 3) or 1 (fp16 x 2)");
    KOAF_REQUIRE(g.A.tf >= 0 && g.A.tf <= 3 && g.B.tf >= 0 && g.B.tf <= 1, "koaf_gemm: tf is 0 | 1 (A, B) | 2 | 3 (A)");
    KOAF_REQUIRE(g.A.tf != 3 || (g.A.kind == 0 && g.A.gather == 0 && g.A.ptr2 && g.A.sc && g.A.sh && g.fmt == 1 && g.B.kind == 2 &&
                                 g.nb0 * g.nb1 == 1 && g.splitk == 1 && aligned16(g.A.ptr2) && (!g.A.side || aligned16(g.A.side)) &&
                                 (!g.A.sc2 || (g.A.sh2 && aligned16(g.A.sc2) && aligned16(g.A.sh2)))),
                 "koaf_gemm: the bottleneck-tail prologue (tf 3) needs a dense K-contiguous A, ptr2 / sc / sh, the fp16 scheme with a pre-split B");
    KOAF_REQUIRE(g.A.tf != 2 || (g.A.ptr2 && g.A.sc && g.A.sh && g.A.sc2 && g.fmt == 1),
                 "koaf_gemm: the two-source prologue needs ptr2 / sc / sh / sc2 and the fp16 scheme");
    if (g.B.kind == 2) {
        KOAF_REQUIRE(g.fmt == 1 && g.B.amax, "koaf_gemm: plane images are fp16 pieces of B * scale(*B.amax): fmt 1, amax required");
        KOAF_REQUIRE((g.A.kind == 0 || g.A.kind == 2) && !g.B.tf, "koaf_gemm: a pre-split B pairs with a K-contiguous A and takes no transform");
    }
    const TilePlan tp = plan_tiles(g);
    const bool vec = tp.vec;
    KOAF_REQUIRE(!g.out_planes || (tp.vec && g.out_sc && g.out_sh && g.ldc == g.N && !(g.N & 7) && g.nb0 * g.nb1 == 1 && g.splitk == 1 && !g.cmap &&
                                   !g.residual && !g.bnb_mode && g.out_ps == (int64_t)g.M * g.N && aligned16(g.out_planes) && aligned16(g.out_sc) &&
                                   aligned16(g.out_sh)),
                 "koaf_gemm: out_planes needs the vector epilogue of a plain forward call (ldc == N, N %% 8 == 0, no batch / split-K / row map / "
                 "residual / BatchNorm-backward), out_ps == M * N and 16-B aligned out_planes / out_sc / out_sh");
    KOAF_REQUIRE(((tp.bm == 64 || tp.bm == 128) && (tp.bn == 64 || tp.bn == 128)) || tp.halo || tp.t2d, "koaf_gemm: tile must be 64|128");
    if (g.A.gather || g.B.gather) KOAF_REQUIRE(vec, "koaf_gemm: gathered operands need aligned, C%%32==0 tensors");
    if (g.B.kind >= 2 || g.A.kind >= 2) KOAF_REQUIRE(vec, "koaf_gemm: pre-split operands need 16-B aligned images (and C %% 32 == 0 per tap)");
    if (g.B.kind == 1 && g.B.gather == 1)
        KOAF_REQUIRE(g.B.C % 4 == 0, "koaf_gemm: gathered K-major operand needs channels per tap (%d) %% 4 == 0", g.B.C);
    KOAF_REQUIRE(!g.cmap || vec, "koaf_gemm: row map needs the vector epilogue");
    KOAF_REQUIRE(!g.bnb_mode || vec, "koaf_gemm: fused BN-backward needs the vector epilogue");
    hipStream_t s = (hipStream_t)stream;
    g.bm = tp.bm;
    g.bn = tp.bn;
    const int64_t tiles = cdiv64(g.M - g.m_base, tp.bm) * cdiv64(g.N, tp.bn);
    if (tiles <= 0) return KOAF_OK;
    if (tiles >= (1ll << 31)) { koaf_set_error("koaf_gemm: grid too large"); return KOAF_EINVAL; }
    dim3 grid((unsigned)tiles, (unsigned)g.splitk, (unsigned)(g.nb0 * g.nb1));
    if (g.act16 < 0 || g.act16 > 3) { koaf_set_error("koaf_gemm: act16 must be 0 .. 3"); return KOAF_EINVAL; }
    return launch_planned(g, tp, grid, s);
}

extern "C" int koaf_slab_reduce(const float* slabs, int32_t nslab, int64_t n, float* out, void* stream) {
    KOAF_REQUIRE(slabs && out && nslab >= 1 && n > 0 && (n & 3) == 0, "koaf_slab_reduce: bad args (n %% 4 == 0)");
    KOAF_REQUIRE((((uintptr_t)slabs | (uintptr_t)out) & 15) == 0, "koaf_slab_reduce: unaligned");
    const unsigned bx = (unsigned)cdiv64(n / 4, 64);
    hipStream_t s = (hipStream_t)stream;
    if (nslab >= 64 && bx < 256) {
        float* part = const_cast<float*>(slabs) + (int64_t)nslab * n;
        hipLaunchKernelGGL(slab_reduce_kernel, dim3(bx, 16), dim3(256), 0, s, slabs, nslab, n, part);
        int rc = koaf_check_launch("koaf_slab_reduce/1");
        if (rc != KOAF_OK) return rc;
        hipLaunchKernelGGL(slab_reduce_kernel, dim3(bx, 1), dim3(256), 0, s, part, 16, n, out);
        return koaf_check_launch("koaf_slab_reduce/2");
    }
    hipLaunchKernelGGL(slab_reduce_kernel, dim3(bx, 1), dim3(256), 0, s, slabs, nslab, n, out);
    return koaf_check_launch("koaf_slab_reduce");
}

extern "C" int koaf_slab_reduce_epilogue(const float* slabs, int32_t nslab, int32_t M, int32_t N, const float* bias,
                                         const float* residual, int64_t ldr, float* out, int64_t ldo, void* stream) {
    KOAF_REQUIRE(slabs && out && nslab >= 1 && M > 0 && N > 0 && (N & 3) == 0 && (ldo & 3) == 0 && (ldr & 3) == 0,
                 "koaf_slab_reduce_epilogue: bad args");
    const int64_t total = (int64_t)M * (N / 4);
    int64_t blocks = cdiv64(total, 256);
    if (blocks > 4096) blocks = 4096;
    hipLaunchKernelGGL(slab_reduce_epi_kernel, dim3((unsigned)blocks), dim3(256), 0, (hipStream_t)stream, slabs, nslab, M,
                       N, bias, residual, ldr, out, ldo);
    return koaf_check_launch("koaf_slab_reduce_epilogue");
}

extern "C" int koaf_set_stream(int on) {
    if (g_stream_mode < 0) { const char* e = getenv("KOAF_STREAM"); g_stream_mode = (e && e[0] == '0') ? 0 : 1; }
    const int was = g_stream_mode;
    g_stream_mode = on ? 1 : 0;
    return was;
}

extern "C" int koaf_launch_log(int on) {
    std::lock_guard<std::mutex> lock(g_log_mutex);
    const int was = g_log_on.load(std::memory_order_relaxed);
    g_log.clear();
    g_log_seen = 0;
    g_log_on.store(on ? 1 : 0, std::memory_order_relaxed);
    return was;
}

extern "C" int koaf_launch_log_read(KoafLaunchRec* out, int32_t cap) {
    std::lock_guard<std::mutex> lock(g_log_mutex);
    for (size_t i = 0; out && i < g_log.size() && (int64_t)i < cap; ++i) out[i] = g_log[i];
    return (int)(g_log_seen < INT32_MAX ? g_log_seen : INT32_MAX);
}

extern "C" int koaf_set_conv3x3_halo(int on) {
    const int was = g_halo_mode;
    g_halo_mode = (on >= 0 && on <= 3) ? on : 1;
    return was;
}
```

### oaprogressionmmf_amd/csrc/koaf_gemm_loaders.h

```cpp
#pragma once
#include "koaf_pieces.h"

namespace {

template <bool H>
__device__ __forceinline__ v4f load4_raw(const float* p, int64_t off) {
    if constexpr (!H) return *(const v4f*)(p + off);
    else {
        const uint2 u = *(const uint2*)(reinterpret_cast<const unsigned short*>(p) + off);
        return (v4f){__uint_as_float(u.x), __uint_as_float(u.y), 0.f, 0.f};
    }
}
enum { M_KC = 0,
       M_KC_G1 = 1,
       M_KC_G2 = 2,
       M_KM = 3,
       M_KM_G1 = 4,
       M_KM_G3 = 5,
       M_PS = 6,
       M_PA1 = 7,
       M_PA2 = 8,
       M_PH = 9,
       M_PK = 10,
       M_PKG = 11,
// ... 226 lines not shown
                        s.vm |= (ok ? 1u : 0u) << i;
                    } else {
#pragma unroll
                        for (int j = 0; j < 4; ++j) {
                            const bool ok = rok && (kk + j) < kend;
                            s.r[i][j] = ptr[ok ? base[i] + k0 + j : 0];
                            s.vm |= (ok ? 1u : 0u) << (4 * i + j);
                        }
                    }
                } else {
                    const bool ok = kok && ((tvm >> i) & 1u);
                    s.r[i] = load4_raw<S16>(ptr, ok ? base[i] + (toff[i] + coff) : 0);
                    if constexpr (TF == 2) s.r2[i] = load4_raw<S2_16>(ptr2, ok ? base[i] + (toff[i] + coff) : 0);
                    s.vm |= (ok ? 1u : 0u) << i;
                }
            }
        } else {
            constexpr int CV = ROWS / 4;
            constexpr int RP = 256 / CV;
            const int kr0 = t / CV;
            int c03 = 0, th3 = 0, tw3 = 0;
            if constexpr (MODE == M_KM_G3) {
                c03 = u_coff; th3 = u_kh; tw3 = u_kw;
                u_coff += BK;
                if (u_coff >= op.C) {
                    u_coff -= op.C;
                    if (++u_kw == op.KW) { u_kw = 0; ++u_kh; }
                }
            }
#pragma unroll
            for (int i = 0; i < NU; ++i) {
                const int k = k0 + kr0 + RP * i;
                bool ok = k < kend;
                int64_t off;
                if constexpr (MODE == M_KM) {
                    off = (int64_t)k * op.ld + col;
                } else if constexpr (MODE == M_KM_G3) {
                    off = (int64_t)(c03 + kr0 + RP * i) * op.ld + th3 * op.tap_stride_h + tw3 * op.tap_stride + col;
                } else {
                    const int sy = gsy[i], sx = gsx[i];
                    ok = ok && (unsigned)sy < (unsigned)op.H && (unsigned)sx < (unsigned)op.W;
                    off = goff[i];
                    int nsx = sx + g_cs;
                    const bool c1 = nsx >= g_sxlim;
                    nsx -= c1 ? g_pws : 0;
                    int nsy = sy + g_bs + (c1 ? op.stride : 0);
                    const bool c2 = nsy >= g_sylim;
                    nsy -= c2 ? g_phs : 0;
                    gsx[i] = nsx;
                    gsy[i] = nsy;
                    goff[i] = off + g_d0 + (c1 ? g_d1 : (int64_t)0) + (c2 ? g_d2 : (int64_t)0);
                }
                if (VEC) {
                    ok = ok && (cvm & 1u);
                    s.r[i] = load4_raw<S16>(ptr, ok ? off : 0);
                    if constexpr (TF == 2) s.r2[i] = load4_raw<S2_16>(ptr2, ok ? off : 0);
                    s.vm |= (ok ? 1u : 0u) << i;
                } else {
#pragma unroll
                    for (int j = 0; j < 4; ++j) {
                        const bool okj = ok && ((cvm >> j) & 1u);
                        s.r[i][j] = ptr[okj ? off + j : 0];
                        s.vm |= (okj ? 1u : 0u) << (4 * i + j);
                    }
                }
            }
        }
    }

    float* side = nullptr;
    int k0s = 0;
    template <bool FULL>
    __device__ __forceinline__ void finish_unit(Slot& s, int i, v4f a, v4f b, v4f k, v4f q = (v4f){0.f, 0.f, 0.f, 0.f}) {
        constexpr float HMAX = 65504.f;
        if constexpr (S16) s.r[i] = widen_bf16x4(__float_as_uint(s.r[i][0]), __float_as_uint(s.r[i][1]));
        if constexpr (S2_16 && (TF == 2 || TF == 3)) s.r2[i < NU2 ? i : 0] = widen_bf16x4(__float_as_uint(s.r2[i < NU2 ? i : 0][0]), __float_as_uint(s.r2[i < NU2 ? i : 0][1]));
#pragma unroll
        for (int j = 0; j < 4; ++j) {
            const bool ok = FULL || (VEC ? ((s.vm >> i) & 1u) : ((s.vm >> (4 * i + j)) & 1u));
            float x = s.r[i][j];
            if constexpr (TF == 1) {
                x = fmaf(x, a[j], b[j]);
                x = F16 ? __builtin_amdgcn_fmed3f(x, 0.f, HMAX) : fmaxf(x, 0.f);
            } else if constexpr (TF == 2) {
                x = fmaf(a[j], x, fmaf(-k[j], s.r2[i < NU2 ? i : 0][j], b[j]));
                if constexpr (F16) x = __builtin_amdgcn_fmed3f(x, -HMAX, HMAX);
            } else if constexpr (TF == 3) {
                float idv = s.r2[i < NU2 ? i : 0][j];
                if (tail2) idv = fmaf(idv, k[j], q[j]);
                x = fmaxf(fmaf(x, a[j], b[j]) + idv, 0.f);
                if constexpr (S16) x = widen_bf16x4(round_bf16x4((v4f){x, 0.f, 0.f, 0.f}).x, 0u)[0];
                s.r2[i < NU2 ? i : 0][j] = x;
                x = fminf(x * fsc, HMAX);
            } else if constexpr (F16) {
                x = __builtin_amdgcn_fmed3f(x * fsc, -HMAX, HMAX);
            }
            s.r[i][j] = ok ? x : 0.f;
        }
        if constexpr (TF == 3) {
            if (side != nullptr && (FULL || ((s.vm >> i) & 1u))) {
                if constexpr (S16) store4<true>(side, base[i] + k0s, s.r2[i < NU2 ? i : 0]);
                else *(v4f*)(side + base[i] + k0s) = s.r2[i < NU2 ? i : 0];
            }
        }
    }
    __device__ __forceinline__ void finish(Slot& s) {
        v4f a = KC ? s.ts4 : kts4, b = KC ? s.th4 : kth4, k = KC ? s.tk4 : ktk4;
        if constexpr (F16 && KC && TF != 0 && TF != 3) { a *= fsc; b *= fsc; k *= fsc; }
        constexpr unsigned ALLV = VEC ? ((NU >= 32) ? ~0u : ((1u << NU) - 1u)) : ((4 * NU >= 32) ? ~0u : ((1u << (4 * NU)) - 1u));
        if (__builtin_amdgcn_ballot_w64(s.vm != ALLV) == 0ull) {
#pragma unroll
            for (int i = 0; i < NU; ++i) finish_unit<true>(s, i, a, b, k, s.tq4);
        } else {
#pragma unroll
            for (int i = 0; i < NU; ++i) finish_unit<false>(s, i, a, b, k, s.tq4);
        }
    }
    __device__ __forceinline__ int plane_off(int i) const {
        const int t = threadIdx.x;
        if constexpr (KC) {
            return ((t >> 3) + 32 * i) * 20 + 2 * (t & 7);
        } else {
            constexpr int CV = ROWS / 4;
            constexpr int RP = 256 / CV;
            return (t / CV + RP * i) * (ROWS / 2 + 16) + 2 * (t % CV);
        }
    }

    template <int NPL>
    __device__ __forceinline__ void store(const Slot& s, float* Sf) {
        unsigned* S = (unsigned*)Sf;
        constexpr int P = plane_dwords(ROWS, KC);
#pragma unroll
        for (int i = 0; i < NU; ++i) {
            unsigned pl[NPL][2];
            if constexpr (F16) split2h(s.r[i], pl);
            else split3v(s.r[i], pl);
            if constexpr (F16 && (TF == 1 || TF == 3) && KC) {
                typedef unsigned short u16x2 __attribute__((ext_vector_type(2)));
#pragma unroll
                for (int d = 0; d < 2; ++d)
                    satmax = __builtin_bit_cast(unsigned, __builtin_elementwise_max(__builtin_bit_cast(u16x2, satmax),
                                                                                     __builtin_bit_cast(u16x2, pl[0][d])));
            }
            const int off = plane_off(i);
#pragma unroll
            for (int q = 0; q < NPL; ++q) *(uint2*)&S[q * P + off] = make_uint2(pl[q][0], pl[q][1]);
        }
    }
};


constexpr int STREAM_TAB_K = 1024;
template <int TF, int SD>
struct StreamA {
    static constexpr bool TWO = (TF == 2 || TF == 3);
    struct Slot {
        v4f r[4];
        v4f r2[TWO ? 4 : 1];
        v4f ts, th, tk, tq;
    };
    Slot sl[SD];
    const float* ptr;
    const float* ptr2;
    const float* sc;
    const float* sh;
    const float* sc2;
    const float* sh2;
    const float* tab;
    int64_t ld;
    float fsc;
    bool tail2;
    bool once;
    unsigned satmax;
    v4l ibase;
    int ik;
    v4l cbase;
    unsigned rvm;
    int kbeg, kend;

    __device__ __forceinline__ v4l bases(int m0, int M) const {
        const int lane = threadIdx.x & 63, w = threadIdx.x >> 6;
        v4l b;
#pragma unroll
        for (int i = 0; i < 4; ++i) {
            const int row = min(m0 + 32 * w + 8 * i + (lane >> 3), M - 1);
            b[i] = (int64_t)row * ld + 4 * (lane & 7);
        }
        return b;
    }
    __device__ __forceinline__ void init(const KoafOperand& op, const float* p, int m0, int M, int kb, int ke, float scale) {
        ptr = p;
        ptr2 = TWO ? op.ptr2 + (p - op.ptr) : nullptr;
        sc = op.sc; sh = op.sh; sc2 = op.sc2; sh2 = op.sh2;
        ld = op.ld;
        fsc = scale;
        tail2 = (TF == 3) && op.sc2 != nullptr;
        once = false;
        satmax = 0u;
        tab = nullptr;
        kbeg = kb; kend = ke;
        ik = kb;
        ibase = bases(m0, M);
        tile(m0, M);
    }
    __device__ __forceinline__ void tile(int m0, int M) {
        const int lane = threadIdx.x & 63, w = threadIdx.x >> 6;
        rvm = 0;
#pragma unroll
        for (int i = 0; i < 4; ++i) rvm |= ((m0 + 32 * w + 8 * i + (lane >> 3)) < M ? 1u : 0u) << i;
        if constexpr (TF == 3) cbase = bases(m0, M);
    }
    template <class NextFn>
    __device__ __forceinline__ void issue(Slot& s, NextFn next, int M) {
        const int lane = threadIdx.x & 63;
        const int c = ik + 4 * (lane & 7);
        if constexpr (TF > 1) {
            s.ts = *(const v4f*)(sc + c);
            s.th = *(const v4f*)(sh + c);
            if constexpr (TF == 2) s.tk = *(const v4f*)(sc2 + c);
            if constexpr (TF == 3) {
                if (tail2) { s.tk = *(const v4f*)(sc2 + c); s.tq = *(const v4f*)(sh2 + c); }
            }
        }
        if (once) {
#pragma unroll
            for (int i = 0; i < 4; ++i) {
                s.r[i] = __builtin_nontemporal_load((const v4f*)(ptr + ibase[i] + ik));
                if constexpr (TWO) s.r2[i] = __builtin_nontemporal_load((const v4f*)(ptr2 + ibase[i] + ik));
            }
        } else {
#pragma unroll
            for (int i = 0; i < 4; ++i) {
                s.r[i] = *(const v4f*)(ptr + ibase[i] + ik);
                if constexpr (TWO) s.r2[i] = *(const v4f*)(ptr2 + ibase[i] + ik);
            }
        }
        ik += BK;
        if (ik >= kend) {
            ik = kbeg;
            const int nm0 = next();
            if (nm0 >= 0) ibase = bases(nm0, M);
        }
    }
    template <bool FULL>
    __device__ __forceinline__ void consume_as(Slot& s, unsigned* S, int k0, float* side) {
        constexpr float HMAX = 65504.f;
        constexpr int P = plane_dwords(128, true);
        const int lane = threadIdx.x & 63, w = threadIdx.x >> 6;
        v4f a = s.ts, b = s.th, k = s.tk;
        if constexpr (TF == 2) { a *= fsc; b *= fsc; k *= fsc; }
        if constexpr (TF == 1) {
            a = *(const v4f*)(tab + (k0 - kbeg) + 4 * (lane & 7));
            b = *(const v4f*)(tab + STREAM_TAB_K + (k0 - kbeg) + 4 * (lane & 7));
        }
#pragma unroll
        for (int i = 0; i < 4; ++i) {
            const bool ok = FULL || ((rvm >> i) & 1u);
            v4f x = s.r[i];
            [[maybe_unused]] v4f y = x;
#pragma unroll
            for (int j = 0; j < 4; ++j) {
                float v = x[j];
                if constexpr (TF == 1) {
                    v = fmaf(v, a[j], b[j]);
                    v = __builtin_amdgcn_fmed3f(v, 0.f, HMAX);
                } else if constexpr (TF == 2) {
                    v = fmaf(a[j], v, fmaf(-k[j], s.r2[i][j], b[j]));
                    v = __builtin_amdgcn_fmed3f(v, -HMAX, HMAX);
                } else if constexpr (TF == 3) {
                    float idv = s.r2[i][j];
                    if (tail2) idv = fmaf(idv, k[j], s.tq[j]);
                    v = fmaxf(fmaf(v, a[j], b[j]) + idv, 0.f);
                    y[j] = v;
                    v = fminf(v * fsc, HMAX);
                } else {
                    v = __builtin_amdgcn_fmed3f(v * fsc, -HMAX, HMAX);
                }
                x[j] = ok ? v : 0.f;
            }
            if constexpr (TF == 3) {
                if (side != nullptr && ok) *(v4f*)(side + cbase[i] + k0) = y;
            }
            unsigned pl[2][2];
            split2h(x, pl);
            if constexpr (TF == 1 || TF == 3) {
                typedef unsigned short u16x2 __attribute__((ext_vector_type(2)));
#pragma unroll
                for (int d = 0; d < 2; ++d)
                    satmax = __builtin_bit_cast(unsigned, __builtin_elementwise_max(__builtin_bit_cast(u16x2, satmax),
                                                                                     __builtin_bit_cast(u16x2, pl[0][d])));
            }
            const int off = (32 * w + 8 * i + (lane >> 3)) * 20 + 2 * (lane & 7);
#pragma unroll
            for (int q = 0; q < 2; ++q) *(uint2*)&S[q * P + off] = make_uint2(pl[q][0], pl[q][1]);
        }
    }
    __device__ __forceinline__ void consume(Slot& s, unsigned* S, int k0, float* side) {
        if (__builtin_amdgcn_ballot_w64(rvm != 15u) == 0ull) consume_as<true>(s, S, k0, side);
        else consume_as<false>(s, S, k0, side);
    }
};

template <int ROWS>
struct PlaneLoader {
    static constexpr int NPIECE = ROWS / 16;
    static constexpr int PPW = NPIECE / 4;
    static constexpr int PLANE_BYTES = ROWS * 64;
    int64_t src[PPW];
    int u_coff, u_kh, u_kw;

    __device__ __forceinline__ void init(const KoafOperand& op, int r0, int R) {
        const int lane = threadIdx.x & 63, w = threadIdx.x >> 6;
#pragma unroll
        for (int j = 0; j < PPW; ++j) {
            const int row = min(r0 + 16 * (w + 4 * j) + (lane >> 2), R - 1);
            src[j] = (int64_t)row * op.ld + 8 * ((lane & 3) ^ ((lane >> 4) & 3));
        }
        u_coff = u_kh = u_kw = 0;
    }
    __device__ __forceinline__ void seek(const KoafOperand& op, int k0) {
        const int tap = k0 / op.C;
        u_coff = k0 - tap * op.C;
        u_kh = tap / op.KW;
        u_kw = tap - u_kh * op.KW;
    }
    template <int NPL>
    __device__ __forceinline__ void issue(const KoafOperand& op, const unsigned short* planes, unsigned lds) {
        const int w = threadIdx.x >> 6;
        const int64_t koff = u_kh * op.tap_stride_h + u_kw * op.tap_stride + u_coff;
        u_coff += BK;
        if (u_coff >= op.C) {
            u_coff -= op.C;
            if (++u_kw == op.KW) { u_kw = 0; ++u_kh; }
        }
#pragma unroll
        for (int q = 0; q < NPL; ++q)
#pragma unroll
            for (int j = 0; j < PPW; ++j)
                lds_dma16(planes + q * op.plane_stride + src[j] + koff, lds + q * PLANE_BYTES + (w + 4 * j) * 1024);
    }
};

template <int ROWS, int G>
struct PlaneGatherLoader {
    static constexpr int NPIECE = ROWS / 16;
    static constexpr int PPW = NPIECE / 4;
    static_assert(PPW >= 1 && PPW <= 4, "1..4 pieces per wave");
// ... 188 lines not shown
```

### oaprogressionmmf_amd/models/_encoder.py

```python
import torch
from torch import nn

from .. import ops
from ..arena import deliver_grad, grad_target, packed_weight, weight_planes
from ._core_fes import BasicBlock, Bottleneck


import os

USE_SIDE_STREAM = os.environ.get("KOAF_SIDE_STREAM", "1") != "0"


class _Rec:
    __slots__ = ("kind", "blk", "yin", "c1", "s1", "c2", "s2", "c3", "s3", "cd", "sd", "y", "dims", "wexp", "tail")

    def __init__(self):
        for k in self.__slots__:
            setattr(self, k, None)


def _stat_shift(bn, train):
    return bn.running_mean if (train and bn is not None and bn.running_mean is not None) else None


FUSE_TAIL = os.environ.get("KOAF_FUSE_TAIL", "1") != "0"
FUSE_TAIL_DS = os.environ.get("KOAF_FUSE_TAIL_DS", "1") != "0"


def _can_take_tail(blk):
    c = getattr(blk, "conv1", None)
    if not (FUSE_TAIL and isinstance(blk, Bottleneck) and c is not None and ops.CONV_F16):
        return False
    if c.kernel_size != (1, 1) or c.stride != (1, 1) or c.groups != 1 or c.in_channels % 32:
        return False
    img = weight_planes(c.weight)
    return img is not None and img[0] is not None


KEEP_PLANES_RECOMPUTE = os.environ.get("KOAF_KEEP_PLANES_RECOMPUTE", "1") != "0"


EMIT_PLANES = os.environ.get("KOAF_EMIT_PLANES", "1") != "0"


def _takes_planes(conv):
    if not (EMIT_PLANES and ops.CONV_F16 and (ops.APLANES_MASK & 1)):
        return False
    if conv.kernel_size != (3, 3) or conv.stride != (1, 1) or conv.groups != 1:
        return False
    img = weight_planes(conv.weight)
    return img is not None and img[0] is not None and ops.use_aplanes(img, 3, 3, conv.in_channels)


def _conv_fwd(x, conv, N, H, W, in_saved, train, bn=None, tail_idt=None, tail_out=None, tail_idsaved=None, keep_planes=False, emit=None):
    w = packed_weight(conv.weight)
    cin, cout = conv.in_channels, conv.out_channels
    k, s, p, g = conv.kernel_size[0], conv.stride[0], conv.padding[0], conv.groups
    sc, sh = (in_saved[2], in_saved[3]) if in_saved is not None else (None, None)
    wexp = None
    shift = _stat_shift(bn, train)
    if tail_idt is not None:
        y, part, yin = ops.conv2d_fwd(x, w, N, H, W, cin, cout, k, k, s, p, sc, sh, stats=train, shift=shift,
                                      wimg=weight_planes(conv.weight), tail_idt=tail_idt, tail_out=tail_out,
                                      tail_idsaved=tail_idsaved, emit=emit)
        return y, part, ops.conv_out(H, k, s, p), ops.conv_out(W, k, s, p), wexp, yin
    if g == 1:
        y, part = ops.conv2d_fwd(x, w, N, H, W, cin, cout, k, k, s, p, sc, sh, stats=train, shift=shift,
                                 wimg=weight_planes(conv.weight), keep_planes=keep_planes, emit=emit)
    else:
        if k != 3 or p != 1 or cin != cout:
            raise NotImplementedError("grouped convolution other than the ResNeXt 3x3 is not built")
        wexp = ops.gconv_expand_w(w, cin, g)
        y, part = ops.gconv3x3_fwd(x, wexp, N, H, W, cin, s, sc, sh, stats=train, shift=shift)
    return y, part, ops.conv_out(H, k, s, p), ops.conv_out(W, k, s, p), wexp


def _bn_fin(bn, part, count):
    train = bn.training or bn.running_mean is None
    return ops.bn_finalize(part if train else None, bn.num_features, count, bn.weight.detach(), bn.bias.detach(),
                           bn.running_mean, bn.running_var, bn.num_batches_tracked if train else None,
                           -1.0 if bn.momentum is None else bn.momentum, bn.eps, train, shift=_stat_shift(bn, train))


_LANES = {}


def lane_streams(device, lane):
    key = (device.index, lane)
    if key not in _LANES:
        hi, lo = _priorities()
        _LANES[key] = (torch.cuda.Stream(device=device, priority=hi), torch.cuda.Stream(device=device, priority=lo))
    return _LANES[key]


def _priorities():
    try:
        lo, hi = torch.cuda.Stream.priority_range()
    except Exception:
        lo, hi = 0, -1
    if os.environ.get("KOAF_STREAM_PRIORITY", "0") == "0":
        return 0, 0
    return hi, lo


_JOIN = {"queued": False, "streams": []}
CALLER_STREAM = None


def _final_join():
    for st, caller in _JOIN["streams"]:
        (caller if caller is not None else torch.cuda.current_stream()).wait_stream(st)
    _JOIN["streams"] = []
    _JOIN["queued"] = False


def _register_join(stream, caller=None):
    _JOIN["streams"].append((stream, caller))
    if not _JOIN["queued"]:
        _JOIN["queued"] = True
        from torch.autograd import Variable
        Variable._execution_engine.queue_callback(_final_join)


class _SideStream:
    _streams = {}

    def __init__(self, device, stream=None, hold=False):
        if stream is None:
            key = (device.type, device.index)
            if key not in _SideStream._streams:
                _SideStream._streams[key] = torch.cuda.Stream(device=device, priority=_priorities()[1])
            stream = _SideStream._streams[key]
        self.stream = stream
        self.pending = []
        self.hold = hold
        self.held = []

    def run(self, inputs, fn, param, buf, acc):
        main = torch.cuda.current_stream()
        self.stream.wait_stream(main)
        with torch.cuda.stream(self.stream):
            fn()
        if self.hold:
            self.held.append(inputs)
        else:
            for t in inputs:
                if t is not None:
                    t.record_stream(self.stream)
        self.pending.append((param, buf, acc))

    def join(self):
        torch.cuda.current_stream().wait_stream(self.stream)
        for param, buf, acc in self.pending:
            deliver_grad(param, buf, acc)
        self.pending = []
        self.held = []


FUSE_APPLY = os.environ.get("KOAF_FUSE_APPLY", "1") != "0"
WGRAD_EARLY = os.environ.get("KOAF_WGRAD_EARLY", "0") == "1"


def _conv_bwd(conv, dc, x, N, H, W, in_saved, wexp, residual=None, need_dx=True, side=None, bnb=None):
    w = packed_weight(conv.weight)
    cin, cout = conv.in_channels, conv.out_channels
    k, s, p, g = conv.kernel_size[0], conv.stride[0], conv.padding[0], conv.groups
    wimg = weight_planes(conv.weight) if g == 1 else None
    if isinstance(dc, ops.BnApply) and (g != 1 or (need_dx and wimg is None)):
        dc = dc.materialize(want_amax=True)
    amax = getattr(dc, "_koaf_amax", None)
    sc, sh = (in_saved[2], in_saved[3]) if in_saved is not None else (None, None)
    gw, acc = grad_target(conv.weight)

    def wgrad():
        if g == 1:
            ops.conv2d_wgrad(dc, x, gw, N, H, W, cin, cout, k, k, s, p, sc, sh, dy_amax=amax)
        else:
            dwexp = ops.gconv3x3_wgrad(dc, x, N, H, W, cin, s, sc, sh)
            ops.gconv_compress_dw(dwexp, gw, cin, g)
    if side is None:
        wgrad()
        deliver_grad(conv.weight, gw, acc)
    early = side is not None and WGRAD_EARLY and need_dx and g == 1 and k == 1
    if early:
        held = dc.tensors() if isinstance(dc, ops.BnApply) else (dc, amax)
        side.run(held + (x, in_saved), wgrad, conv.weight, gw, acc)
    dx = None
    if need_dx:
        if g == 1:
            dx = ops.conv2d_dgrad(dc, w, N, H, W, cin, cout, k, k, s, p, residual=residual, bnb=bnb, wimg=wimg, dy_amax=amax)
        else:
            assert residual is None and bnb is None
            dx = ops.gconv3x3_dgrad(dc, wexp, N, H, W, cin, s)
    if side is not None and not early:
        held = dc.tensors() if isinstance(dc, ops.BnApply) else (dc, amax)
        side.run(held + (x, in_saved), wgrad, conv.weight, gw, acc)
    return dx


def _bn_bwd(bn, g, c, saved, rows, mask_mode, ymask=None, dz_out=None, dc_out=None, fused=None, pool=None):
    C = bn.num_features
    gg, ag = grad_target(bn.weight)
    gb, ab = grad_target(bn.bias)
    if fused is None:
        fused = ops.CONV_F16
        dc = ops.bn_bwd(g, c, saved, rows, C, rows, gg, gb, mask_mode, ymask=ymask, dz_out=dz_out, fused=fused)
        if fused and not FUSE_APPLY:
            dc = dc.materialize(out=dc_out, want_amax=True)
    else:
        dc = ops.bn_bwd(g, c, saved, rows, C, rows, gg, gb, mask_mode, ymask=ymask, dz_out=dz_out,
                        dc_out=None if fused else dc_out, fused=fused, pool=pool)
    deliver_grad(bn.weight, gg, ag)
    deliver_grad(bn.bias, gb, ab)
    return dc


def _bn_bwd_part(bn, part, nsum, i1, dz, c, saved, rows, dc_out=None, dzmax=None):
    C = bn.num_features
    gg, ag = grad_target(bn.weight)
    gb, ab = grad_target(bn.bias)
    fused = ops.CONV_F16 and dzmax is not None
    dc = ops.bn_bwd_from_part(part, nsum, i1, dz, c, saved, rows, C, rows, gg, gb, dc_out=None if fused else dc_out,
                              fused=fused, dzmax=dzmax)
    if fused and not FUSE_APPLY:
        dc = dc.materialize(out=dc_out, want_amax=True)
    deliver_grad(bn.weight, gg, ag)
    deliver_grad(bn.bias, gb, ab)
    return dc


FUSE_BNB = os.environ.get("KOAF_FUSE_BNB", "1") != "0"
FUSE_STEM_BWD = os.environ.get("KOAF_FUSE_STEM_BWD", "1") != "0"
REUSE_STAGE_INPUT = os.environ.get("KOAF_REUSE_STAGE_INPUT", "1") != "0"


def _tail_bnb(prev):
    if prev is None or not FUSE_BNB:
        return None
    c_last, s_last = (prev.c3, prev.s3) if prev.kind == "bottleneck" else (prev.c2, prev.s2)
    d = dict(mode=1, c=c_last, y=prev.y, saved=s_last, dz_amax=ops.CONV_F16)
    if prev.cd is not None:
        d["c2"], d["saved2"] = prev.cd, prev.sd
    return d


def _block_fwd(blk, y, N, Hc, Wc, train, given, tail=None, defer=False, skip_tail=False):
    r = _Rec()
    r.blk, r.yin = blk, y
    want = train and given is None

    def fin(bn, part, count, idx):
        return given[idx] if given is not None else _bn_fin(bn, part, count)
    if isinstance(blk, Bottleneck):
        r.kind = "bottleneck"
        s1_pre, emit = None, None
        if not want and _takes_planes(blk.conv2) and blk.conv1.groups == 1 and weight_planes(blk.conv1.weight) is not None:
            s1_pre = fin(blk.bn1, None, N * Hc * Wc, 0)
            emit = (s1_pre[2], s1_pre[3])
        if tail is not None:
            r.c1, part, _, _, _, y = _conv_fwd(tail[0], blk.conv1, N, Hc, Wc, tail[1], want, blk.bn1, tail_idt=tail[2], tail_out=tail[3],
                                               tail_idsaved=tail[4], emit=emit)
            r.yin = y
        else:
            r.c1, part, _, _, _ = _conv_fwd(y, blk.conv1, N, Hc, Wc, None, want, blk.bn1, emit=emit)
        r.s1 = s1_pre if s1_pre is not None else fin(blk.bn1, part, N * Hc * Wc, 0)
        r.c2, part, OH, OW, r.wexp = _conv_fwd(r.c1, blk.conv2, N, Hc, Wc, r.s1, want, blk.bn2,
                                               keep_planes=given is not None and KEEP_PLANES_RECOMPUTE)
        r.s2 = fin(blk.bn2, part, N * OH * OW, 1)
        r.c3, part, _, _, _ = _conv_fwd(r.c2, blk.conv3, N, OH, OW, r.s2, want, blk.bn3)
        r.s3 = fin(blk.bn3, part, N * OH * OW, 2)
        last_c, last_s, cout = r.c3, r.s3, blk.conv3.out_channels
    elif isinstance(blk, BasicBlock):
        r.kind = "basic"
        r.c1, part, OH, OW, _ = _conv_fwd(y, blk.conv1, N, Hc, Wc, None, want, blk.bn1)
        r.s1 = fin(blk.bn1, part, N * OH * OW, 0)
        r.c2, part, _, _, _ = _conv_fwd(r.c1, blk.conv2, N, OH, OW, r.s1, want, blk.bn2)
        r.s2 = fin(blk.bn2, part, N * OH * OW, 1)
        last_c, last_s, cout = r.c2, r.s2, blk.conv2.out_channels
    else:
        raise TypeError(f"unsupported block {type(blk)}")
    rows_o = N * OH * OW
    if blk.downsample is not None:
        r.cd, part, _, _, _ = _conv_fwd(y, blk.downsample[0], N, Hc, Wc, None, want, blk.downsample[1])
        r.sd = fin(blk.downsample[1], part, rows_o, 3)
        if skip_tail:
            pass
        elif defer and FUSE_TAIL_DS:
            r.tail = (last_c, last_s, r.cd, torch.empty_like(last_c), r.sd)
        else:
            r.y = ops.bn_add_relu(last_c, last_s, rows_o, cout, idt=r.cd, idsaved=r.sd)
    elif skip_tail:
        pass
    elif defer:
        r.tail = (last_c, last_s, y, torch.empty_like(last_c), None)
    else:
        r.y = ops.bn_add_relu(last_c, last_s, rows_o, cout, idt=y)
    r.dims = (N, Hc, Wc, OH, OW)
    return r


def _blocks_fwd(blocks, y, N, Hc, Wc, train, givens=None, tail=None, defer_last=False, slim=False, last_y=None):
    recs, yin0 = [], None
    for i, blk in enumerate(blocks):
        nxt = blocks[i + 1] if i + 1 < len(blocks) else None
        defer = (nxt is not None and _can_take_tail(nxt)) or (nxt is None and defer_last)
        have = nxt is None and last_y is not None
        r = _block_fwd(blk, y, N, Hc, Wc, train, givens[i] if givens is not None else None, tail=tail, defer=defer, skip_tail=have)
        if have:
            r.y = last_y
        if i == 0:
            yin0 = r.yin
        if recs:
            if tail is not None:
                recs[-1].y = r.yin
            if slim:
                p = recs[-1]
                p.c1 = p.c2 = p.c3 = p.cd = p.y = p.yin = p.tail = p.wexp = None
        recs.append(r)
        y, Hc, Wc = r.y, r.dims[3], r.dims[4]
        tail = r.tail
    return recs, y, Hc, Wc, yin0


def _recompute_plan(trunk, nstages):
    r = getattr(trunk, "recompute", False)
    if r is False or r is None:
        return frozenset(), False
    if r is True or r == "stage":
        return frozenset(range(nstages)), False
    if r == "block":
        return frozenset(range(nstages)), True
    rs = frozenset(int(i) for i in r)
    if not rs <= frozenset(range(nstages)):
        raise ValueError(f"KoafTrunk.recompute: stage indices out of range 0..{nstages - 1}: {sorted(rs)}")
    return rs, False


class EncoderFn(torch.autograd.Function):
    @staticmethod
    def forward(ctx, x, trunk, anchor, keep, lane):
        st = trunk._koaf_layout()
        if x.dim() == 4:
            if x.shape[1] != 1:
                raise ValueError("KoafTrunk takes the single-channel image (the 1->3 repeat is folded into conv1)")
            N, _, H, W = x.shape
        else:
            N, H, W = x.shape
        x = x.contiguous()
        conv1, bn1 = st["conv1"], st["bn1"]
        train = bn1.training
        w1t = ops.stem_fold_w(packed_weight(conv1.weight))
        adt = getattr(trunk, "act_dtype", torch.float32)
        if train:
            c0, part = ops.stem_fwd(x, w1t, N, H, W, dtype=adt, stats=True, shift=_stat_shift(bn1, train))
        else:
            c0, part = ops.stem_fwd(x, w1t, N, H, W, dtype=adt), None
        H1, W1 = c0.shape[1], c0.shape[2]
        s0 = _bn_fin(bn1, part, N * H1 * W1)
        y, am = ops.maxpool_fwd(c0, s0, N, H1, W1, 64)
        Hc, Wc = y.shape[1], y.shape[2]
        rset, block_level = _recompute_plan(trunk, len(st["stages"]))
        if not keep:
            rset = frozenset()
        stages_saved = []
        tail, prev_recs = None, None
        nst = len(st["stages"])
        for si, stage in enumerate(st["stages"]):
            rec_stage = si in rset
            defer_last = si + 1 < nst and _can_take_tail(st["stages"][si + 1][0])
            recs, y_out, Ho, Wo, yin0 = _blocks_fwd(stage, y, N, Hc, Wc, train, tail=tail, defer_last=defer_last, slim=rec_stage or not keep)
            if tail is not None:
                y = yin0
                if prev_recs:
                    prev_recs[-1].y = y
            sv = dict(yin=y if rec_stage else None, H=Hc, W=Wc, stats=[], recs=[], recompute=rec_stage)
            if rec_stage:
                sv["stats"] = [(r.s1, r.s2, r.s3, r.sd) for r in recs]
            elif keep:
                sv["recs"] = recs
            tail = recs[-1].tail
            prev_recs = sv["recs"]
            if rec_stage or not keep:
                for r in recs:
                    r.c1 = r.c2 = r.c3 = r.cd = r.yin = r.y = None
            del recs
            y, Hc, Wc = y_out, Ho, Wo
            stages_saved.append(sv)
        C = y.shape[-1]
        if st["gap"]:
            out = ops.gap_fwd(y, N, Hc * Wc, C).view(N, C, 1, 1)
        else:
            out = y.permute(0, 3, 1, 2)
            if out.dtype != torch.float32:
                out = out.float()
        if keep:
            if 0 in rset:
                c0 = None
            ctx.state = dict(x=x, c0=c0, s0=s0, am=am, stages=stages_saved, any_recompute=bool(rset), caller=CALLER_STREAM,
                             block_level=block_level, adt=adt,
                             dims=(N, H, W, H1, W1), last=(Hc, Wc, C), st=st, lane=lane, train=train)
        return out

    @staticmethod
    def backward(ctx, gout):
        S = ctx.state
        ctx.state = None
        lane = S["lane"]
        if lane is None:
            return EncoderFn._backward_body(S, gout, None)
        main_s, side_s = lane_streams(gout.device, lane)
        cur = torch.cuda.current_stream()
        if cur != main_s:
            main_s.wait_stream(cur)
            gout.record_stream(main_s)
        with torch.cuda.stream(main_s):
            out = EncoderFn._backward_body(S, gout, side_s)
        _register_join(main_s, S.get("caller"))
        return out

    @staticmethod
    def _blocks_bwd(recs, dy, side):
        pend = None
        while recs:
            r = recs.pop()
            prev = recs[-1] if recs else None
            blk = r.blk
            N, Hi, Wi, OH, OW = r.dims
            rows_o, rows_i = N * OH * OW, N * Hi * Wi
            bott = r.kind == "bottleneck"
            tail_bn = blk.bn3 if bott else blk.bn2
            tail_c, tail_s = (r.c3, r.s3) if bott else (r.c2, r.s2)
            if pend is None:
                dcl = _bn_bwd(tail_bn, dy, tail_c, tail_s, rows_o, 1, ymask=r.y, dz_out=dy)
            else:
                dcl = _bn_bwd_part(tail_bn, pend[0], pend[1], 1, dy, tail_c, tail_s, rows_o, dzmax=pend[2])
            dz = dy
            inner = FUSE_BNB
            want_max = ops.CONV_F16

            def split(res):
                return res if len(res) == 3 else (res[0], res[1], None)
            if bott:
                g2 = blk.conv2.groups == 1 and inner
                res = _conv_bwd(blk.conv3, dcl, r.c2, N, OH, OW, r.s2, None, side=side,
                                bnb=dict(mode=2, c=r.c2, saved=r.s2, dz_amax=want_max) if inner else None)
                del dcl
                if inner:
                    da2, part2, mx2 = split(res)
                    dc2 = _bn_bwd_part(blk.bn2, part2, 2, 1, da2, r.c2, r.s2, rows_o, dc_out=da2, dzmax=mx2)
                else:
                    da2 = res
                    dc2 = _bn_bwd(blk.bn2, da2, r.c2, r.s2, rows_o, 2, dc_out=da2)
                res = _conv_bwd(blk.conv2, dc2, r.c1, N, Hi, Wi, r.s1, r.wexp, side=side,
                                bnb=dict(mode=2, c=r.c1, saved=r.s1, dz_amax=want_max) if g2 else None)
                del dc2, da2
                if g2:
                    da1, part1, mx1 = split(res)
                    dc1 = _bn_bwd_part(blk.bn1, part1, 2, 1, da1, r.c1, r.s1, rows_i, dc_out=da1, dzmax=mx1)
                else:
                    da1 = res
                    dc1 = _bn_bwd(blk.bn1, da1, r.c1, r.s1, rows_i, 2, dc_out=da1)
            else:
                res = _conv_bwd(blk.conv2, dcl, r.c1, N, OH, OW, r.s1, None, side=side,
                                bnb=dict(mode=2, c=r.c1, saved=r.s1, dz_amax=want_max) if inner else None)
                del dcl
                if inner:
                    da1, part1, mx1 = split(res)
                    dc1 = _bn_bwd_part(blk.bn1, part1, 2, 1, da1, r.c1, r.s1, rows_o, dc_out=da1, dzmax=mx1)
                else:
                    da1 = res
                    dc1 = _bn_bwd(blk.bn1, da1, r.c1, r.s1, rows_o, 2, dc_out=da1)
            first = blk.conv1
            if blk.downsample is not None:
                if pend is None:
                    dcd = _bn_bwd(blk.downsample[1], dz, r.cd, r.sd, rows_o, 0, dc_out=dz)
                else:
                    dcd = _bn_bwd_part(blk.downsample[1], pend[0], pend[1], 2, dz, r.cd, r.sd, rows_o, dc_out=dz, dzmax=pend[2])
                resid = _conv_bwd(blk.downsample[0], dcd, r.yin, N, Hi, Wi, None, None, side=side)
            else:
                resid = dz
            bnb = _tail_bnb(prev)
            res = _conv_bwd(first, dc1, r.yin, N, Hi, Wi, None, None, residual=resid, side=side, bnb=bnb)
            if bnb is not None:
                dy, part, mx = split(res)
                pend = (part, 3 if "c2" in bnb else 2, mx)
            else:
                dy, pend = res, None
            del dc1, da1, dz, resid, r
            if side is not None and side.hold:
                side.join()
        return dy

    @staticmethod
    def _backward_body(S, gout, side_stream):
        st = S["st"]
        N, H, W, H1, W1 = S["dims"]
        Hc, Wc, C = S["last"]
        if st["gap"]:
            dy = ops.gap_bwd(gout.reshape(N, C).contiguous(), N, Hc * Wc, C).view(N, Hc, Wc, C)
        else:
            dy = gout.permute(0, 2, 3, 1).contiguous()
            if dy.data_ptr() == gout.data_ptr():
                dy = dy.clone()
        side = _SideStream(gout.device, side_stream, hold=S["any_recompute"]) if USE_SIDE_STREAM else None
        stages = st["stages"]
        run = []
        next_in = None
        for si in range(len(stages) - 1, -1, -1):
            sv = S["stages"][si]
            if not sv["recompute"]:
                run = sv["recs"] + run
                sv["recs"] = None
                if si > 0 and not S["stages"][si - 1]["recompute"]:
                    continue
                first_in = run[0].yin if REUSE_STAGE_INPUT else None
                dy = EncoderFn._blocks_bwd(run, dy, side)
                run = []
                next_in = first_in
                continue
            y, Hc2, Wc2 = sv["yin"], sv["H"], sv["W"]
            sv["yin"] = None
            stage_in, last_y = (y if REUSE_STAGE_INPUT else None), next_in
            next_in = None
            if S["block_level"] and len(stages[si]) > 1:
                ins = [(y, Hc2, Wc2)]
                for blk, given in zip(stages[si][:-1], sv["stats"][:-1]):
                    r = _block_fwd(blk, y, N, Hc2, Wc2, S["train"], given)
                    y, Hc2, Wc2 = r.y, r.dims[3], r.dims[4]
                    ins.append((y, Hc2, Wc2))
                    del r
                for bi in range(len(stages[si]) - 1, -1, -1):
                    yb, hb, wb = ins.pop()
                    r = _block_fwd(stages[si][bi], yb, N, hb, wb, S["train"], sv["stats"][bi])
                    dy = EncoderFn._blocks_bwd([r], dy, side)
                    del r, yb
                del y, last_y
                next_in = stage_in
                continue
            recs, y, Hc2, Wc2, _ = _blocks_fwd(stages[si], y, N, Hc2, Wc2, S["train"], givens=sv["stats"], last_y=last_y)
            del last_y
            dy = EncoderFn._blocks_bwd(recs, dy, side)
            del recs, y
            next_in = stage_in
        next_in = None
        conv1, bn1 = st["conv1"], st["bn1"]
        c0 = S["c0"]
        if c0 is None:
            c0 = ops.stem_fwd(S["x"], ops.stem_fold_w(packed_weight(conv1.weight)), N, H, W, dtype=S["adt"])
        if FUSE_STEM_BWD:
            dc0 = _bn_bwd(bn1, None, c0, S["s0"], N * H1 * W1, 2, fused=True, pool=(dy, S["am"], N, H1, W1))
        else:
            da0 = ops.maxpool_bwd(dy, S["am"], N, H1, W1, 64)
            dc0 = _bn_bwd(bn1, da0, c0, S["s0"], N * H1 * W1, 2, dc_out=da0, fused=False)
        gw, acc = grad_target(conv1.weight)
        ops.stem_wgrad(dc0, S["x"], gw, N, H, W)
        deliver_grad(conv1.weight, gw, acc)
        if side is not None:
            side.join()
        return None, None, None, None, None


class KoafTrunk(nn.Sequential):
    act_dtype = torch.float32

    def _koaf_layout(self):
        lay = self.__dict__.get("_koaf_lay")
        if lay is not None:
            return lay
        ch = list(self.children())
        if not (len(ch) >= 8 and isinstance(ch[0], nn.Conv2d) and isinstance(ch[1], nn.BatchNorm2d)
                and isinstance(ch[3], nn.MaxPool2d)):
            raise TypeError("KoafTrunk expects the children of a koaf ResNet (conv1, bn1, relu, maxpool, layer1-4[, avgpool])")
        c1 = ch[0]
        if c1.kernel_size != (7, 7) or c1.stride != (2, 2) or c1.padding != (3, 3) or c1.out_channels != 64:
            raise NotImplementedError("stem other than 7x7/s2/p3 -> 64 is not built")
        blocks, stages = [], []
        gap = False
        for m in ch[4:]:
            if isinstance(m, nn.Sequential):
                blocks.extend(list(m.children()))
                stages.append(list(m.children()))
            elif isinstance(m, nn.AdaptiveAvgPool2d):
                gap = True
            else:
                raise TypeError(f"unexpected trunk child {type(m)}")
        lay = dict(conv1=ch[0], bn1=ch[1], blocks=blocks, stages=stages, gap=gap)
        self.__dict__["_koaf_lay"] = lay
        return lay

    def forward(self, x, lane=None):
        lay = self._koaf_layout()
        anchor = lay["conv1"].weight
        keep = torch.is_grad_enabled() and anchor.requires_grad
        return EncoderFn.apply(x, self, anchor, keep, lane)
```

### oaprogressionmmf_amd/ops.py

```python
import ctypes

import torch

from ._lib import KoafBnApply, KoafBnb, KoafEmit, KoafGemm, KoafError, KoafLaunchRec, KoafTail, KoafWImg, check, lib

_i32 = ctypes.c_int32

import os
CONV_F16 = os.environ.get("KOAF_CONV_FMT", "f16") != "bf16"
APLANES_MASK = int(os.environ.get("KOAF_APLANES", "7"))
APLANES = APLANES_MASK != 0
ACT_SCALE = 16.0
KEEP_XPLANES_ELEMS = int(os.environ.get("KOAF_KEEP_XPLANES_ELEMS", "0"))

PROFILE = None


def _prof_begin():
    if PROFILE is None:
        return None
    e = torch.cuda.Event(enable_timing=True)
    e.record()
    return e


def _prof_end(e0, family, flops, tag="", elems=0, mpp=6):
    if e0 is None:
        return
    e1 = torch.cuda.Event(enable_timing=True)
    e1.record()
    PROFILE.append((family, flops, e0, e1, tag, 4.0 * elems, mpp))


def _ptr(t):
    if t is None:
        return None
    if not t.is_cuda:
        raise KoafError("koaf ops need tensors on a HIP device (no CPU fallback exists)")
    if t.dtype not in (torch.float32, torch.int64, torch.uint8, torch.float64, torch.bfloat16):
        raise KoafError(f"unexpected dtype {t.dtype}")
    return t.data_ptr()


_STATUS = None
_STATUS_DEV = None


def _a16(t):
    return 1 if (t is not None and t.dtype == torch.bfloat16) else 0


def _stream():
    if _STATUS is None or _STATUS_DEV != torch.cuda.current_device():
        _status_buffer()
    return torch.cuda.current_stream().cuda_stream


_STATUS_BY_DEV = {}


def _status_buffer():
    global _STATUS, _STATUS_DEV
    d = torch.cuda.current_device()
    if _STATUS is None or _STATUS_DEV != d:
        if d not in _STATUS_BY_DEV:
            _STATUS_BY_DEV[d] = torch.zeros(4, dtype=torch.int32, device=torch.device("cuda", d))
        _STATUS, _STATUS_DEV = _STATUS_BY_DEV[d], d
        check(lib().koaf_set_status_buffer(_STATUS.data_ptr()), "set_status_buffer")
    return _STATUS


def numerics_status(reset=False):
    st = _status_buffer()
    torch.cuda.synchronize(st.device)
    v = st.cpu().tolist()
    if reset:
        st.zero_()
    return {"saturated": int(v[0]) & 0xffffffff, "nonfinite": int(v[1]) & 0xffffffff}


def check_numerics(reset=True):
    import warnings
    st = numerics_status(reset=reset)
    if st["saturated"]:
        warnings.warn(f"koaf: {st['saturated']} activation elements / tiles exceeded the fixed activation scale's range (|x| > 4094 behind "
                      f"a BatchNorm) and were clamped in the convolution operands: results are no longer at fp32 rounding level",
                      RuntimeWarning, stacklevel=2)
    if st["nonfinite"]:
        warnings.warn(f"koaf: non-finite values reached {st['nonfinite']} operand scales / BatchNorm coefficients (a diverged run)",
                      RuntimeWarning, stacklevel=2)
    return st


def _img(wimg):
    if wimg is None:
        return None
    f, d, amax = wimg
    for t in (f, d):
        if t is not None and (not t.is_cuda or t.dtype != torch.int16):
            raise KoafError("weight plane images are int16 (fp16 bit patterns) tensors on the HIP device")
    return ctypes.byref(KoafWImg(f=f.data_ptr() if f is not None else None, d=d.data_ptr() if d is not None else None,
                                 amax=_ptr(amax)))


class BnApply(object):
    __slots__ = ("dz", "c", "coef", "amax", "mean", "rows", "C", "_koaf_planes")

    def __init__(self, dz, c, coef, amax, mean, rows, C):
        self.dz, self.c, self.coef, self.amax, self.mean, self.rows, self.C = dz, c, coef, amax, mean, rows, C
        self._koaf_planes = None

    def struct(self):
        return ctypes.byref(KoafBnApply(dz=_ptr(self.dz), c=_ptr(self.c), coef=_ptr(self.coef), amax=_ptr(self.amax)))

    def tensors(self):
        return (self.dz, self.c, self.coef, self.amax, self._koaf_planes, getattr(self.c, "_koaf_xplanes", None))

    def materialize(self, out=None, want_amax=False):
        dc = out if out is not None else torch.empty(self.c.shape, device=self.c.device, dtype=torch.float32)
        amax = torch.zeros(1, device=self.c.device, dtype=torch.float32) if want_amax else None
        check(lib().koaf_bn_bwd_apply(_ptr(self.dz), _ptr(self.c), _ptr(self.mean), _ptr(self.coef), _ptr(dc), self.rows, self.C,
                                      _ptr(amax), _a16(self.c), _stream()), "bn_bwd_apply")
        if want_amax:
            dc._koaf_amax = amax
        return dc


def _dy_args(dy, dy_amax):
    if isinstance(dy, BnApply):
        return None, None, dy.struct(), dy.dz
    return _ptr(dy), _ptr(dy_amax), None, dy


def _empty(shape, like, dtype=torch.float32):
    return torch.empty(shape, device=like.device, dtype=dtype)


def conv_out(h, k, s, p):
    return (h + 2 * p - k) // s + 1


def act_planes(x, npix, C, tf=0, sc=None, sh=None, x2=None, sc2=None, amax=None, fscale=0.0):
    L = lib()
    out = torch.empty(L.koaf_act_planes_elems(npix, C), device=x.device, dtype=torch.int16)
    check(L.koaf_act_planes(_ptr(x), _ptr(x2), npix, C, tf, _ptr(sc), _ptr(sh), _ptr(sc2), _ptr(amax), float(fscale),
                            out.data_ptr(), _a16(x2 if tf == 2 else x), _stream()), "act_planes")
    return out


def set_conv3x3_halo(mode):
    return lib().koaf_set_conv3x3_halo(int(mode))


def set_stream(on):
    return bool(lib().koaf_set_stream(1 if on else 0))


def launch_log(on):
    return bool(lib().koaf_launch_log(1 if on else 0))


def launch_log_read():
    L = lib()
    n = min(L.koaf_launch_log_read(None, 0), 4096)
    buf = (KoafLaunchRec * max(n, 1))()
    L.koaf_launch_log_read(buf, n)
    return [{f: (getattr(r, f).decode() if f == "variant" else getattr(r, f)) for f, _ in KoafLaunchRec._fields_} for r in buf[:n]]


def use_aplanes(wimg, KH, KW, C):
    return APLANES and wimg is not None and KH * KW > 1 and C % 32 == 0


def conv2d_fwd(x, w, N, H, W, Cin, Cout, KH, KW, stride, pad, in_sc=None, in_sh=None, stats=False, shift=None, wimg=None,
               aplanes=None, tail_idt=None, tail_out=None, tail_idsaved=None, keep_planes=False, emit=None):
    L = lib()
    OH, OW = conv_out(H, KH, stride, pad), conv_out(W, KW, stride, pad)
    if tail_idt is not None and tail_out is None:
        tail_out = torch.empty_like(x)
    y = _empty((N, OH, OW, Cout), x, dtype=x.dtype)
    part, rows = None, _i32(0)
    if stats:
        nrows = L.koaf_conv2d_stats_rows(N * OH * OW, Cout)
        part = _empty((nrows, 2, Cout), x)
    e0 = _prof_begin()
    if aplanes is None:
        aplanes = (APLANES_MASK & 1) and use_aplanes(wimg, KH, KW, Cin) and wimg[0] is not None and stride == 1
    xpl = None
    tail = None
    if tail_idt is not None:
        tail = ctypes.byref(KoafTail(idt=_ptr(tail_idt), y_out=_ptr(tail_out),
                                     idt_sc=_ptr(tail_idsaved[2]) if tail_idsaved is not None else None,
                                     idt_sh=_ptr(tail_idsaved[3]) if tail_idsaved is not None else None))
        aplanes = False
    if torch.is_tensor(aplanes):
        xpl = aplanes
    elif aplanes:
        ep = getattr(x, "_koaf_eplanes", None)
        if ep is not None:
            del x._koaf_eplanes
        if (ep is not None and in_sc is not None and ep[1].data_ptr() == in_sc.data_ptr() and ep[2].data_ptr() == in_sh.data_ptr()
                and ep[0].numel() == L.koaf_act_planes_elems(N * H * W, Cin)):
            xpl = ep[0]
        else:
            xpl = act_planes(x, N * H * W, Cin, 1 if in_sc is not None else 0, in_sc, in_sh, fscale=ACT_SCALE)
    epl, em = None, None
    if emit is not None:
        epl = torch.empty(L.koaf_act_planes_elems(N * OH * OW, Cout), device=x.device, dtype=torch.int16)
        em = ctypes.byref(KoafEmit(planes=epl.data_ptr(), sc=_ptr(emit[0]), sh=_ptr(emit[1])))
    check(L.koaf_conv2d_fwd(_ptr(x), _ptr(w), _ptr(y), N, H, W, Cin, Cout, KH, KW, stride, pad, _ptr(in_sc),
                            _ptr(in_sh), _ptr(part), ctypes.addressof(rows), _ptr(shift) if stats else None,
                            _img(wimg), xpl.data_ptr() if xpl is not None else None, tail, em, _a16(x), _stream()), "conv2d_fwd")
    if epl is not None:
        y._koaf_eplanes = (epl, emit[0], emit[1])
    if xpl is not None and not torch.is_tensor(aplanes) and (keep_planes or xpl.numel() <= KEEP_XPLANES_ELEMS):
        y._koaf_xplanes = xpl
    _prof_end(e0, "gemm", 2.0 * N * OH * OW * Cout * KH * KW * Cin,
              f"conv_fwd k{KH}s{stride} {Cin}->{Cout} px{N*OH*OW}" + (" +tail" if tail is not None else ""),
              N * H * W * Cin * (3 if tail is not None else 1) + Cout * KH * KW * Cin + N * OH * OW * Cout * (2 if epl is not None else 1),
              mpp=3 if wimg is not None else 6)
    if stats:
        part = part[:rows.value]
    if tail is not None:
        return y, part, tail_out
    return y, part


def conv2d_dgrad(dy, w, N, H, W, Cin, Cout, KH, KW, stride, pad, residual=None, bnb=None, wimg=None, dy_amax=None,
                 aplanes=None):
    L = lib()
    dyp, amp, app, like = _dy_args(dy, dy_amax)
    a16 = _a16(dy.c) if isinstance(dy, BnApply) else (_a16(bnb["c"]) if bnb is not None else 0)
    dx = _empty((N, H, W, Cin), like)
    if aplanes is None:
        aplanes = ((APLANES_MASK & 2) and use_aplanes(wimg, KH, KW, Cout) and wimg[1] is not None and stride in (1, 2) and
                   (app is not None or dy_amax is not None))
    e0 = _prof_begin()
    dypl = None
    if aplanes:
        dypl = _dy_planes(dy, dy_amax, N * conv_out(H, KH, stride, pad) * conv_out(W, KW, stride, pad), Cout)
    dypp = dypl.data_ptr() if dypl is not None else None
    fl = 2.0 * N * conv_out(H, KH, stride, pad) * conv_out(W, KW, stride, pad) * Cout * KH * KW * Cin
    tag = f"conv_dgrad k{KH}s{stride} {Cin}->{Cout} px{N*H*W}"
    el = N * conv_out(H, KH, stride, pad) * conv_out(W, KW, stride, pad) * Cout + Cout * KH * KW * Cin + N * H * W * Cin
    el += N * H * W * Cin if residual is not None else 0
    mpp = 3 if (wimg is not None and (dy_amax is not None or app is not None)) else 6
    if app is not None:
        el += N * conv_out(H, KH, stride, pad) * conv_out(W, KW, stride, pad) * Cout
        tag += " apply"
    if bnb is None:
        check(L.koaf_conv2d_dgrad(dyp, _ptr(w), _ptr(dx), N, H, W, Cin, Cout, KH, KW, stride, pad,
                                  _ptr(residual), _img(wimg), amp, app, dypp, a16, _stream()), "conv2d_dgrad")
        _prof_end(e0, "gemm", fl, tag, el, mpp=mpp)
        return dx
    sv, sv2 = bnb["saved"], bnb.get("saved2")
    dzmax = _empty((1,), like) if bnb.get("dz_amax") else None
    kb = KoafBnb(mode=bnb["mode"], dz_amax=_ptr(dzmax), c=_ptr(bnb["c"]), y=_ptr(bnb.get("y")), sc=_ptr(sv[2]), sh=_ptr(sv[3]),
                 mean=_ptr(sv[0]), invstd=_ptr(sv[1]), c2=_ptr(bnb.get("c2")),
                 mean2=_ptr(sv2[0]) if sv2 is not None else None, invstd2=_ptr(sv2[1]) if sv2 is not None else None)
    nsum = 3 if bnb.get("c2") is not None else 2
    part = _empty((L.koaf_conv2d_dgrad_bnb_rows(N, H, W, Cin, stride), nsum, Cin), like)
    rows = _i32(0)
    check(L.koaf_conv2d_dgrad_bnb(dyp, _ptr(w), _ptr(dx), N, H, W, Cin, Cout, KH, KW, stride, pad,
                                  _ptr(residual), ctypes.byref(kb), _ptr(part), ctypes.addressof(rows), _img(wimg),
                                  amp, app, dypp, a16, _stream()), "conv2d_dgrad_bnb")
    el += N * H * W * Cin * (1 + (bnb.get("y") is not None) + (bnb.get("c2") is not None))
    _prof_end(e0, "gemm", fl, tag + " +bnb", el, mpp=mpp)
    if dzmax is not None:
        return dx, part[:rows.value], dzmax
    return dx, part[:rows.value]


def _dy_planes(dy, dy_amax, npo, Cout):
    if isinstance(dy, BnApply):
        if dy._koaf_planes is None:
            dy._koaf_planes = act_planes(dy.dz, npo, Cout, 2, dy.coef[0], dy.coef[3], x2=dy.c, sc2=dy.coef[2], amax=dy.amax)
        return dy._koaf_planes
    return act_planes(dy, npo, Cout, 0, amax=dy_amax)


def conv2d_wgrad(dy, x, dw, N, H, W, Cin, Cout, KH, KW, stride, pad, in_sc=None, in_sh=None, dy_amax=None, aplanes=None):
    L = lib()
    dyp, amp, app, like = _dy_args(dy, dy_amax)
    ws = L.koaf_conv2d_wgrad_ws(N, H, W, Cin, Cout, KH, KW, stride, pad)
    slabs = _empty((ws,), like) if ws > 0 else None
    if aplanes is None:
        aplanes = ((APLANES_MASK & 4) and KH * KW > 1 and stride == 1 and Cin % 8 == 0 and Cout % 8 == 0 and
                   (app is not None or dy_amax is not None))
    e0 = _prof_begin()
    dypl = xpl = None
    if aplanes:
        npo = N * conv_out(H, KH, stride, pad) * conv_out(W, KW, stride, pad)
        dypl = _dy_planes(dy, dy_amax, npo, Cout)
        xpl = getattr(dy.c, "_koaf_xplanes", None) if app is not None else None
        if xpl is None or xpl.numel() != L.koaf_act_planes_elems(N * H * W, Cin):
            xpl = act_planes(x, N * H * W, Cin, 1 if in_sc is not None else 0, in_sc, in_sh, fscale=ACT_SCALE)
    check(L.koaf_conv2d_wgrad(dyp, _ptr(x), _ptr(dw), N, H, W, Cin, Cout, KH, KW, stride, pad, _ptr(in_sc),
                              _ptr(in_sh), _ptr(slabs), amp, app, dypl.data_ptr() if dypl is not None else None,
                              xpl.data_ptr() if xpl is not None else None, _a16(x), _stream()), "conv2d_wgrad")
    npx = N * conv_out(H, KH, stride, pad) * conv_out(W, KW, stride, pad)
    _prof_end(e0, "gemm", 2.0 * npx * Cout * KH * KW * Cin,
              f"conv_wgrad k{KH}s{stride} {Cin}->{Cout} px{N*H*W}" + (" apply" if app is not None else ""),
              npx * Cout * (2 if app is not None else 1) + N * H * W * Cin + Cout * KH * KW * Cin,
              mpp=3 if (dy_amax is not None or app is not None) else 6)
    return dw


def gconv_expand_w(w, C, groups):
    wexp = _empty((C // 64, 64, 9, 64), w)
    amax = torch.zeros(1, device=w.device, dtype=torch.float32) if CONV_F16 else None
    check(lib().koaf_gconv_expand_w(_ptr(w), _ptr(wexp), C, groups, _ptr(amax), _stream()), "gconv_expand_w")
    if amax is not None:
        wexp._koaf_amax = amax
    return wexp


def gconv_compress_dw(dwexp, dw, C, groups):
    check(lib().koaf_gconv_compress_dw(_ptr(dwexp), _ptr(dw), C, groups, _stream()), "gconv_compress_dw")
    return dw


def gconv3x3_fwd(x, wexp, N, H, W, C, stride, in_sc=None, in_sh=None, stats=False, shift=None):
    L = lib()
    OH, OW = conv_out(H, 3, stride, 1), conv_out(W, 3, stride, 1)
    y = _empty((N, OH, OW, C), x, dtype=x.dtype)
    part, rows = None, _i32(0)
    if stats:
        part = _empty(((N * OH * OW + 127) // 128, 2, C), x)
    e0 = _prof_begin()
    wam = getattr(wexp, "_koaf_amax", None)
    check(L.koaf_gconv3x3_fwd(_ptr(x), _ptr(wexp), _ptr(y), N, H, W, C, stride, _ptr(in_sc), _ptr(in_sh), _ptr(part),
                              ctypes.addressof(rows), _ptr(shift) if stats else None, _ptr(wam), _a16(x), _stream()), "gconv3x3_fwd")
    _prof_end(e0, "gemm", 2.0 * N * OH * OW * C * 9 * (C // 32), f"gconv_fwd s{stride} C{C} px{N*OH*OW}",
              N * H * W * C + N * OH * OW * C + 9 * C * (C // 32), mpp=3 if (wam is not None and not _a16(x)) else 6)
    return y, part


def gconv3x3_dgrad(dy, wexp, N, H, W, C, stride):
    dx = _empty((N, H, W, C), dy)
    e0 = _prof_begin()
    wam, dam = getattr(wexp, "_koaf_amax", None), getattr(dy, "_koaf_amax", None)
    if wam is None or dam is None:
        wam = dam = None
    check(lib().koaf_gconv3x3_dgrad(_ptr(dy), _ptr(wexp), _ptr(dx), N, H, W, C, stride, _ptr(wam), _ptr(dam), _stream()), "gconv3x3_dgrad")
    _prof_end(e0, "gemm", 2.0 * N * conv_out(H, 3, stride, 1) * conv_out(W, 3, stride, 1) * C * 9 * (C // 32),
              f"gconv_dgrad s{stride} C{C} px{N*H*W}",
              N * H * W * C + N * conv_out(H, 3, stride, 1) * conv_out(W, 3, stride, 1) * C + 9 * C * (C // 32), mpp=3 if wam is not None else 6)
    return dx


def gconv3x3_wgrad(dy, x, N, H, W, C, stride, in_sc=None, in_sh=None):
    L = lib()
    ws = L.koaf_gconv3x3_wgrad_ws(N, H, W, C, stride)
    slabs = _empty((ws,), dy)
    dwexp = _empty((C // 64, 64, 9, 64), dy)
    e0 = _prof_begin()
    dam = getattr(dy, "_koaf_amax", None) if CONV_F16 else None
    check(L.koaf_gconv3x3_wgrad(_ptr(dy), _ptr(x), _ptr(dwexp), N, H, W, C, stride, _ptr(in_sc), _ptr(in_sh),
                                _ptr(slabs), _ptr(dam), _a16(x), _stream()), "gconv3x3_wgrad")
    _prof_end(e0, "gemm", 2.0 * N * conv_out(H, 3, stride, 1) * conv_out(W, 3, stride, 1) * C * 9 * (C // 32),
              f"gconv_wgrad s{stride} C{C} px{N*H*W}",
              N * H * W * C + N * conv_out(H, 3, stride, 1) * conv_out(W, 3, stride, 1) * C + 9 * C * (C // 32),
              mpp=3 if (dam is not None and not _a16(x)) else 6)
    return dwexp


def stem_fold_w(w):
    w1t = _empty((49, 64), w)
    check(lib().koaf_stem_fold_w(_ptr(w), _ptr(w1t), _stream()), "stem_fold_w")
    return w1t


def stem_fwd(x, w1t, N, H, W, dtype=torch.float32, stats=False, shift=None):
    L = lib()
    y = _empty((N, conv_out(H, 7, 2, 3), conv_out(W, 7, 2, 3), 64), x, dtype=dtype)
    part = _empty((L.koaf_stem_stats_rows(N, H), 2, 64), x) if stats else None
    check(L.koaf_stem_fwd(_ptr(x), _ptr(w1t), _ptr(y), N, H, W, _ptr(part), _ptr(shift) if stats else None, _a16(y), _stream()), "stem_fwd")
    return (y, part) if stats else y


def stem_wgrad(dy, x, dw, N, H, W):
    L = lib()
    dyp, _, app, like = _dy_args(dy, None)
    slabs = _empty((L.koaf_stem_wgrad_ws(N, H, W),), like)
    dw1t = _empty((49, 64), like)
    check(L.koaf_stem_wgrad(dyp, _ptr(x), _ptr(dw1t), N, H, W, _ptr(slabs), app, _a16(dy.c) if app is not None else 0, _stream()),
          "stem_wgrad")
    check(L.koaf_stem_unfold_dw(_ptr(dw1t), _ptr(dw), _stream()), "stem_unfold_dw")
    return dw


def colstats(x, rows, C, shift=None):
    L = lib()
    part = _empty((L.koaf_colpart_rows(rows, C), 2, C), x)
    r = _i32(0)
    check(L.koaf_colstats(_ptr(x), rows, C, _ptr(part), ctypes.addressof(r), _ptr(shift), _a16(x), _stream()), "colstats")
    return part


def _reduce_ws(rows, C, like):
    n = lib().koaf_bn_reduce_ws(rows, C)
    return torch.empty(n // 8, dtype=torch.float64, device=like.device) if n else None


def bn_finalize(part, C, count, gamma, beta, running_mean, running_var, nbt, momentum, eps, train, shift=None):
    saved = _empty((4, C), gamma if gamma is not None else running_mean)
    rows = part.shape[0] if part is not None else 0
    ws = _reduce_ws(rows, C, saved) if train else None
    check(lib().koaf_bn_finalize(_ptr(part), rows, C, count, _ptr(gamma), _ptr(beta), _ptr(running_mean),
                                 _ptr(running_var), _ptr(nbt), momentum, eps, 1 if train else 0, _ptr(saved[0]),
                                 _ptr(saved[1]), _ptr(saved[2]), _ptr(saved[3]), _ptr(shift) if train else None, _ptr(ws),
                                 _stream()), "bn_finalize")
    return saved


def bn_add_relu(c, saved, rows, C, idt=None, idsaved=None, out=None):
    y = out if out is not None else torch.empty_like(c)
    check(lib().koaf_bn_add_relu(_ptr(c), _ptr(saved[2]), _ptr(saved[3]), _ptr(idt),
# ... 299 lines not shown
```

Baseline: 4.089 knees/s.

## Route stride-2 1x1 shortcut convs through streamed GEMM and accumulate downsample dgrad

```diff
diff --git a/include/koaf.h b/include/koaf.h
--- a/include/koaf.h
+++ b/include/koaf.h
@@ -26,7 +26,7 @@
     int32_t PH, PW;
     int32_t KH, KW, stride, pad;
     int32_t pad_w;
-    int32_t _pad1;
+    int32_t rowmap;
     int32_t tf;
     int32_t tf_bs;
     const float* sc;
@@ -147,7 +147,8 @@
 int koaf_conv2d_dgrad(const float* dy, const float* w, float* dx, int32_t N, int32_t H, int32_t W,
                       int32_t Cin, int32_t Cout, int32_t KH, int32_t KW, int32_t stride,
                       int32_t pad, const float* residual, const KoafWImg* wimg, const float* dy_amax,
-                      const KoafBnApply* dy_apply, const uint16_t* dy_planes, int32_t act16, void* stream);
+                      const KoafBnApply* dy_apply, const uint16_t* dy_planes, int32_t act16, int32_t accumulate,
+                      void* stream);
 typedef struct KoafBnb {
     int32_t mode, _pad;
     float* dz_amax;
@@ -166,7 +167,7 @@
                           int32_t Cin, int32_t Cout, int32_t KH, int32_t KW, int32_t stride, int32_t pad,
                           const float* residual, const KoafBnb* bnb, float* part, int32_t* part_rows,
                           const KoafWImg* wimg, const float* dy_amax, const KoafBnApply* dy_apply,
-                          const uint16_t* dy_planes, int32_t act16, void* stream);
+                          const uint16_t* dy_planes, int32_t act16, int32_t accumulate, void* stream);
 int64_t koaf_conv2d_wgrad_ws(int32_t N, int32_t H, int32_t W, int32_t Cin, int32_t Cout,
                              int32_t KH, int32_t KW, int32_t stride, int32_t pad);
 int koaf_conv2d_wgrad(const float* dy, const float* x, float* dw, int32_t N, int32_t H, int32_t W,
diff --git a/oaprogressionmmf_amd/_lib.py b/oaprogressionmmf_amd/_lib.py
--- a/oaprogressionmmf_amd/_lib.py
+++ b/oaprogressionmmf_amd/_lib.py
@@ -29,7 +29,7 @@
         ("stride", ctypes.c_int32),
         ("pad", ctypes.c_int32),
         ("pad_w", ctypes.c_int32),
-        ("_pad1", ctypes.c_int32),
+        ("rowmap", ctypes.c_int32),
         ("tf", ctypes.c_int32),
         ("tf_bs", ctypes.c_int32),
         ("sc", ctypes.c_void_p),
@@ -231,6 +231,11 @@
     return protos
 
 
+def header_version(path=HEADER):
+    m = re.search(r"(\d+) = this header", Path(path).read_text())
+    return int(m.group(1)) if m else None
+
+
 _LIB = None
 
 
@@ -248,6 +253,10 @@
             f"libkoaf.so not found at {path}: build it with `python -c 'import __graft_entry__ as g; "
             f"g.build()'` or `make -C oaprogressionmmf_amd/csrc` -- there is no CPU fallback")
     handle = ctypes.CDLL(str(path))
+    want = header_version()
+    if want is not None and hasattr(handle, "koaf_version") and handle.koaf_version() != want:
+        raise KoafError(f"{path} is version {handle.koaf_version()}, include/koaf.h is {want}: rebuild it "
+                        f"(`make -C oaprogressionmmf_amd/csrc`)")
     for name, (restype, argtypes) in parse_header().items():
         fn = getattr(handle, name)
         fn.restype = restype
diff --git a/oaprogressionmmf_amd/csrc/koaf_common.h b/oaprogressionmmf_amd/csrc/koaf_common.h
--- a/oaprogressionmmf_amd/csrc/koaf_common.h
+++ b/oaprogressionmmf_amd/csrc/koaf_common.h
@@ -66,6 +66,9 @@
 __device__ __forceinline__ void block_amax_raise(float v, float* slot) { block_amax_raise_bits(koaf_absbits(v), slot); }
 
 uint32_t* koaf_status_ptr();
+bool koaf_stream_enabled();
+bool koaf_stream_shortcuts();
+bool koaf_gemm_streams(const KoafGemm* g);
 __device__ __forceinline__ void koaf_status_add(uint32_t* st, int slot, unsigned n) {
     if (st != nullptr && n != 0u) atomicAdd(&st[slot], n);
 }
diff --git a/oaprogressionmmf_amd/csrc/koaf_conv.hip b/oaprogressionmmf_amd/csrc/koaf_conv.hip
--- a/oaprogressionmmf_amd/csrc/koaf_conv.hip
+++ b/oaprogressionmmf_amd/csrc/koaf_conv.hip
@@ -271,25 +271,35 @@
     const int64_t M = (int64_t)N * OH * OW;
     KOAF_REQUIRE(M < (1ll << 31), "koaf_conv2d_fwd: too many output pixels");
     KoafGemm g;
-    zero_gemm(&g);
-    g.A.ptr = x;
-    g.A.kind = 0;
-    if (KH == 1 && KW == 1 && stride == 1 && pad == 0 && !x_planes) {
-        g.A.gather = 0;
-        g.A.ld = Cin;
-    } else {
-        g.A.gather = 1;
-        g.A.H = H; g.A.W = W; g.A.C = Cin; g.A.CS = Cin;
-        g.A.PH = OH; g.A.PW = OW;
-        g.A.KH = KH; g.A.KW = KW; g.A.stride = stride; g.A.pad = pad; g.A.pad_w = pad;
-    }
-    if (in_sc) { g.A.tf = 1; g.A.sc = in_sc; g.A.sh = in_sh; }
-    if (tail) { g.A.tf = 3; g.A.ptr2 = tail->idt; g.A.side = tail->y_out; g.A.sc2 = tail->idt_sc; g.A.sh2 = tail->idt_sc ? tail->idt_sh : nullptr; }
-    g.B.ptr = w;
-    g.B.kind = 0;
-    g.B.ld = (int64_t)KH * KW * Cin;
-    g.M = (int)M; g.N = Cout; g.K = KH * KW * Cin;
-    if (wimg && wimg->amax) set_fimg(&g, wimg, Cout, g.K);
+    auto describe = [&](bool mapped) {
+        zero_gemm(&g);
+        g.A.ptr = x;
+        g.A.kind = 0;
+        if (KH == 1 && KW == 1 && stride == 1 && pad == 0 && !x_planes) {
+            g.A.gather = 0;
+            g.A.ld = Cin;
+        } else if (mapped) {
+            g.A.gather = 0;
+            g.A.ld = Cin;
+            g.A.rowmap = 1;
+            g.A.H = H; g.A.W = W; g.A.PH = OH; g.A.PW = OW; g.A.stride = stride;
+        } else {
+            g.A.gather = 1;
+            g.A.H = H; g.A.W = W; g.A.C = Cin; g.A.CS = Cin;
+            g.A.PH = OH; g.A.PW = OW;
+            g.A.KH = KH; g.A.KW = KW; g.A.stride = stride; g.A.pad = pad; g.A.pad_w = pad;
+        }
+        if (in_sc) { g.A.tf = 1; g.A.sc = in_sc; g.A.sh = in_sh; }
+        if (tail) { g.A.tf = 3; g.A.ptr2 = tail->idt; g.A.side = tail->y_out; g.A.sc2 = tail->idt_sc; g.A.sh2 = tail->idt_sc ? tail->idt_sh : nullptr; }
+        g.B.ptr = w;
+        g.B.kind = 0;
+        g.B.ld = (int64_t)KH * KW * Cin;
+        g.M = (int)M; g.N = Cout; g.K = KH * KW * Cin;
+        if (wimg && wimg->amax) set_fimg(&g, wimg, Cout, g.K);
+        g.act16 = act16 ? 1 : 0;
+    };
+    describe(KH == 1 && KW == 1 && stride == 2 && pad == 0 && !x_planes && koaf_stream_shortcuts());
+    if (g.A.rowmap && !koaf_gemm_streams(&g)) describe(false);
     if (x_planes) {
         KOAF_REQUIRE(g.A.gather == 1 && g.B.kind == 2, "koaf_conv2d_fwd: x_planes serve the gathered kernels and need wimg->f");
         set_aplanes(&g.A, x_planes, (int64_t)N * H * W * Cin);
@@ -297,7 +307,6 @@
     g.C = y; g.ldc = Cout;
     g.stats = stats;
     g.stats_shift = stats ? stats_shift : nullptr;
-    g.act16 = act16 ? 1 : 0;
     if (emit) {
         KOAF_REQUIRE(emit->planes && emit->sc && emit->sh && (Cout % 8) == 0, "koaf_conv2d_fwd: emit needs planes / sc / sh and Cout %% 8 == 0");
         g.out_planes = emit->planes; g.out_sc = emit->sc; g.out_sh = emit->sh; g.out_ps = M * Cout;
@@ -338,12 +347,15 @@
                                      int32_t Cin, int32_t Cout, int32_t KH, int32_t KW, int32_t stride, int32_t pad,
                                      const float* residual, const KoafBnb* bnb, float* part, int32_t* part_rows,
                                      const KoafWImg* wimg, const float* dy_amax, const KoafBnApply* dy_apply,
-                                     const uint16_t* dy_planes, int32_t act16, void* stream) {
+                                     const uint16_t* dy_planes, int32_t act16, int32_t accumulate, void* stream) {
     KOAF_REQUIRE(!dy_planes || (wimg && wimg->amax && wimg->d && (dy_amax || dy_apply) && KH * KW > 1),
                  "koaf_conv2d_dgrad: dy_planes need the weight's D plane image, dy_amax and a gathered (KH*KW > 1) kernel");
     KOAF_REQUIRE((dy || dy_apply || dy_planes) && w && dx && N > 0 && Cout % 32 == 0 && Cin % 4 == 0, "koaf_conv2d_dgrad: bad args");
     KOAF_REQUIRE(!dy_apply || (dy_apply->dz && dy_apply->c && dy_apply->coef && dy_apply->amax && wimg && wimg->amax && wimg->d),
                  "koaf_conv2d_dgrad: dy_apply needs dz / c / coef / amax and the weight's D plane image");
+    const bool shortcut = stride == 2 && KH == 1 && KW == 1 && pad == 0;
+    KOAF_REQUIRE(!accumulate || (shortcut && !residual && !bnb),
+                 "koaf_conv2d_dgrad: accumulate serves 1x1 / stride-2 / pad-0 convolutions without residual / fused reduction");
     if (dy_apply) { dy = dy_apply->dz; dy_amax = dy_apply->amax; }
     if (bnb && bnb->dz_amax && hipMemsetAsync(bnb->dz_amax, 0, sizeof(float), (hipStream_t)stream) != hipSuccess) {
         koaf_set_error("koaf_conv2d_dgrad_bnb: memset failed");
@@ -365,29 +377,37 @@
             for (int px = 0; px < 2; ++px) {
                 const int Hc = (H - py + 1) / 2, Wc = (W - px + 1) / 2;
                 if (Hc <= 0 || Wc <= 0) continue;
+                if (accumulate && (py | px)) continue;
                 const int khs = (py + pad) & 1, kws = (px + pad) & 1;
                 const int nkh = khs < KH ? (KH - khs + 1) / 2 : 0, nkw = kws < KW ? (KW - kws + 1) / 2 : 0;
                 const int offy = (py + pad - khs) / 2, offx = (px + pad - kws) / 2;
                 zero_gemm(&g);
                 g.prec = 1;
                 if (f16) { g.fmt = 1; g.A.amax = dy_amax; g.B.amax = wimg->amax; }
-                g.A.ptr = dy; g.A.kind = 0; g.A.gather = 2;
+                g.A.ptr = dy; g.A.kind = 0;
                 if (dy_apply) set_apply(&g.A, dy_apply, Cout);
-                g.A.H = OH; g.A.W = OW; g.A.C = Cout; g.A.CS = Cout;
-                g.A.PH = Hc; g.A.PW = Wc;
-                g.A.KH = nkh > 0 ? nkh : 1; g.A.KW = nkw > 0 ? nkw : 1; g.A.stride = 1; g.A.pad = offy; g.A.pad_w = offx;
-                g.B.ptr = w + ((int64_t)khs * KW + kws) * Cin; g.B.kind = 1; g.B.gather = 3;
-                g.B.C = Cout; g.B.ld = (int64_t)KH * KW * Cin;
-                g.B.KW = g.A.KW; g.B.tap_stride = 2ll * Cin; g.B.tap_stride_h = 2ll * KW * Cin;
-                if (ps) {
-                    g.B.kind = 2; g.B.gather = 0;
-                    g.B.planes = w_dimg + ((int64_t)khs * KW + kws) * Cout; g.B.ld = dld; g.B.plane_stride = dps;
-                    g.B.tap_stride = 2ll * Cout; g.B.tap_stride_h = 2ll * KW * Cout;
+                if (shortcut && !(py | px) && koaf_stream_shortcuts()) {
+                    g.A.gather = 0; g.A.ld = Cout;
+                    g.B.ptr = w; g.B.kind = 1; g.B.gather = 0; g.B.ld = Cin;
+                    if (ps) { g.B.kind = 2; g.B.planes = w_dimg; g.B.ld = dld; g.B.plane_stride = dps; }
+                } else {
+                    g.A.gather = 2;
+                    g.A.H = OH; g.A.W = OW; g.A.C = Cout; g.A.CS = Cout;
+                    g.A.PH = Hc; g.A.PW = Wc;
+                    g.A.KH = nkh > 0 ? nkh : 1; g.A.KW = nkw > 0 ? nkw : 1; g.A.stride = 1; g.A.pad = offy; g.A.pad_w = offx;
+                    g.B.ptr = w + ((int64_t)khs * KW + kws) * Cin; g.B.kind = 1; g.B.gather = 3;
+                    g.B.C = Cout; g.B.ld = (int64_t)KH * KW * Cin;
+                    g.B.KW = g.A.KW; g.B.tap_stride = 2ll * Cin; g.B.tap_stride_h = 2ll * KW * Cin;
+                    if (ps) {
+                        g.B.kind = 2; g.B.gather = 0;
+                        g.B.planes = w_dimg + ((int64_t)khs * KW + kws) * Cout; g.B.ld = dld; g.B.plane_stride = dps;
+                        g.B.tap_stride = 2ll * Cout; g.B.tap_stride_h = 2ll * KW * Cout;
+                    }
                 }
                 if (dy_planes && nkh > 0 && nkw > 0) set_aplanes(&g.A, dy_planes, (int64_t)N * OH * OW * Cout);
                 g.M = N * Hc * Wc; g.N = Cin; g.K = nkh * nkw * Cout;
                 g.C = dx; g.ldc = Cin;
-                g.residual = residual; g.ldr = Cin;
+                g.residual = accumulate ? dx : residual; g.ldr = Cin;
                 g.cmap = 1; g.cm_PH = Hc; g.cm_PW = Wc; g.cm_H = H; g.cm_W = W; g.cm_py = py; g.cm_px = px;
                 if (bnb) {
                     set_bnb(&g, bnb, part + (int64_t)rows_done * nsum * Cin);
@@ -444,9 +464,10 @@
 extern "C" int koaf_conv2d_dgrad(const float* dy, const float* w, float* dx, int32_t N, int32_t H, int32_t W,
                                  int32_t Cin, int32_t Cout, int32_t KH, int32_t KW, int32_t stride, int32_t pad,
                                  const float* residual, const KoafWImg* wimg, const float* dy_amax,
-                                 const KoafBnApply* dy_apply, const uint16_t* dy_planes, int32_t act16, void* stream) {
+                                 const KoafBnApply* dy_apply, const uint16_t* dy_planes, int32_t act16, int32_t accumulate,
+                                 void* stream) {
     return koaf_conv2d_dgrad_bnb(dy, w, dx, N, H, W, Cin, Cout, KH, KW, stride, pad, residual, nullptr, nullptr,
-                                 nullptr, wimg, dy_amax, dy_apply, dy_planes, act16, stream);
+                                 nullptr, wimg, dy_amax, dy_apply, dy_planes, act16, accumulate, stream);
 }
 
 bool koaf_wgrad3_ring_ok(int N, int H, int W, int Cin, int Cout);
diff --git a/oaprogressionmmf_amd/csrc/koaf_elem.hip b/oaprogressionmmf_amd/csrc/koaf_elem.hip
--- a/oaprogressionmmf_amd/csrc/koaf_elem.hip
+++ b/oaprogressionmmf_amd/csrc/koaf_elem.hip
@@ -13,7 +13,7 @@
 static uint32_t* g_status = nullptr;
 uint32_t* koaf_status_ptr() { return g_status; }
 extern "C" int koaf_set_status_buffer(uint32_t* dev4) { g_status = dev4; return KOAF_OK; }
-extern "C" int koaf_version(void) { return 190; }
+extern "C" int koaf_version(void) { return 200; }
 
 namespace {
 
diff --git a/oaprogressionmmf_amd/csrc/koaf_gemm.hip b/oaprogressionmmf_amd/csrc/koaf_gemm.hip
--- a/oaprogressionmmf_amd/csrc/koaf_gemm.hip
+++ b/oaprogressionmmf_amd/csrc/koaf_gemm.hip
@@ -101,9 +101,16 @@
 
 namespace {
 int g_stream_mode = -1;
+int stream_mode() {
+    if (g_stream_mode < 0) { const char* e = getenv("KOAF_STREAM"); g_stream_mode = (e && e[0] == '0') ? 0 : ((e && e[0] == '1') ? 1 : 2); }
+    return g_stream_mode;
+}
+}
+bool koaf_stream_enabled() { return stream_mode() >= 1; }
+bool koaf_stream_shortcuts() { return stream_mode() == 2; }
+namespace {
 bool stream_ok(const KoafGemm& g) {
-    if (g_stream_mode < 0) { const char* e = getenv("KOAF_STREAM"); g_stream_mode = (e && e[0] == '0') ? 0 : 1; }
-    return g_stream_mode == 1 && g.A.kind == 0 && g.A.gather == 0 && g.K >= 2 * BK && (g.K % (2 * BK)) == 0 && g.splitk == 1 &&
+    return koaf_stream_enabled() && g.A.kind == 0 && g.A.gather == 0 && g.K >= 2 * BK && (g.K % (2 * BK)) == 0 && g.splitk == 1 &&
            g.nb0 * g.nb1 == 1 && (g.A.tf != 1 || g.K <= STREAM_TAB_K);
 }
 }
@@ -222,6 +229,12 @@
     }
     return rc;
 }
+}
+
+bool koaf_gemm_streams(const KoafGemm* gp) {
+    KoafGemm g = *gp;
+    fill_defaults(g);
+    return plan_tiles(g).stream && g.A.tf != 3;
 }
 
 extern "C" int koaf_gemm_part_rows(const KoafGemm* gp) {
@@ -271,6 +284,12 @@
     }
     const TilePlan tp = plan_tiles(g);
     const bool vec = tp.vec;
+    KOAF_REQUIRE(!g.A.rowmap || (tp.stream && g.A.tf != 3 && g.A.H > 0 && g.A.W > 0 && g.A.PH > 0 && g.A.PW > 0 && g.A.stride > 0 &&
+                                 (g.M % (g.A.PH * g.A.PW)) == 0 && (g.A.PH - 1) * g.A.stride < g.A.H && (g.A.PW - 1) * g.A.stride < g.A.W &&
+                                 g.A.PH < 16384 && g.A.PW < 16384 && g.A.H < 65536 && g.A.W < 65536 && g.A.stride < 16 && (int64_t)(g.M / (g.A.PH * g.A.PW)) * g.A.H * g.A.W < (1ll << 31)),
+                 "koaf_gemm: A.rowmap is read by the streamed kernel only (koaf.h koaf_set_stream), over a PH x PW grid (< 16384 each) inside "
+                 "H x W, fewer than 2^31 source pixels");
+    KOAF_REQUIRE(!g.B.rowmap, "koaf_gemm: rowmap is an A-operand field");
     KOAF_REQUIRE(!g.out_planes || (tp.vec && g.out_sc && g.out_sh && g.ldc == g.N && !(g.N & 7) && g.nb0 * g.nb1 == 1 && g.splitk == 1 && !g.cmap &&
                                    !g.residual && !g.bnb_mode && g.out_ps == (int64_t)g.M * g.N && aligned16(g.out_planes) && aligned16(g.out_sc) &&
                                    aligned16(g.out_sh)),
@@ -324,9 +343,8 @@
 }
 
 extern "C" int koaf_set_stream(int on) {
-    if (g_stream_mode < 0) { const char* e = getenv("KOAF_STREAM"); g_stream_mode = (e && e[0] == '0') ? 0 : 1; }
-    const int was = g_stream_mode;
-    g_stream_mode = on ? 1 : 0;
+    const int was = stream_mode();
+    g_stream_mode = on <= 0 ? 0 : (on == 1 ? 1 : 2);
     return was;
 }
 
diff --git a/oaprogressionmmf_amd/csrc/koaf_gemm_loaders.h b/oaprogressionmmf_amd/csrc/koaf_gemm_loaders.h
--- a/oaprogressionmmf_amd/csrc/koaf_gemm_loaders.h
+++ b/oaprogressionmmf_amd/csrc/koaf_gemm_loaders.h
@@ -402,6 +402,19 @@
 
 
 constexpr int STREAM_TAB_K = 1024;
+__device__ __attribute__((noinline)) v4l stream_map_rows(unsigned mp_grid, unsigned mp_src, int64_t ld, int m0, int M) {
+    const int lane = threadIdx.x & 63, w = threadIdx.x >> 6;
+    const int ph = mp_grid & 0x3fff, pw = (mp_grid >> 14) & 0x3fff, s = mp_grid >> 28, hh = mp_src & 0xffff, ww = mp_src >> 16;
+    v4l b;
+#pragma unroll
+    for (int i = 0; i < 4; ++i) {
+        const int row = min(m0 + 32 * w + 8 * i + (lane >> 3), M - 1);
+        const int n = row / (ph * pw), rem = row - n * (ph * pw);
+        const int yy = rem / pw, xx = rem - yy * pw;
+        b[i] = (int64_t)((n * hh + s * yy) * ww + s * xx) * ld + 4 * (lane & 7);
+    }
+    return b;
+}
 template <int TF, int SD>
 struct StreamA {
     static constexpr bool TWO = (TF == 2 || TF == 3);
@@ -419,6 +432,7 @@
     const float* sh2;
     const float* tab;
     int64_t ld;
+    unsigned mp_grid, mp_src;
     float fsc;
     bool tail2;
     bool once;
@@ -437,6 +451,7 @@
             const int row = min(m0 + 32 * w + 8 * i + (lane >> 3), M - 1);
             b[i] = (int64_t)row * ld + 4 * (lane & 7);
         }
+        if (mp_grid) b = stream_map_rows(mp_grid, mp_src, ld, m0, M);
         return b;
     }
     __device__ __forceinline__ void init(const KoafOperand& op, const float* p, int m0, int M, int kb, int ke, float scale) {
@@ -444,6 +459,8 @@
         ptr2 = TWO ? op.ptr2 + (p - op.ptr) : nullptr;
         sc = op.sc; sh = op.sh; sc2 = op.sc2; sh2 = op.sh2;
         ld = op.ld;
+        mp_grid = op.rowmap ? ((unsigned)op.PH | (unsigned)op.PW << 14 | (unsigned)op.stride << 28) : 0u;
+        mp_src = (unsigned)op.H | (unsigned)op.W << 16;
         fsc = scale;
         tail2 = (TF == 3) && op.sc2 != nullptr;
         once = false;
diff --git a/oaprogressionmmf_amd/models/_encoder.py b/oaprogressionmmf_amd/models/_encoder.py
--- a/oaprogressionmmf_amd/models/_encoder.py
+++ b/oaprogressionmmf_amd/models/_encoder.py
@@ -161,7 +161,7 @@
 WGRAD_EARLY = os.environ.get("KOAF_WGRAD_EARLY", "0") == "1"
 
 
-def _conv_bwd(conv, dc, x, N, H, W, in_saved, wexp, residual=None, need_dx=True, side=None, bnb=None):
+def _conv_bwd(conv, dc, x, N, H, W, in_saved, wexp, residual=None, need_dx=True, side=None, bnb=None, accumulate=None):
     w = packed_weight(conv.weight)
     cin, cout = conv.in_channels, conv.out_channels
     k, s, p, g = conv.kernel_size[0], conv.stride[0], conv.padding[0], conv.groups
@@ -188,7 +188,8 @@
     dx = None
     if need_dx:
         if g == 1:
-            dx = ops.conv2d_dgrad(dc, w, N, H, W, cin, cout, k, k, s, p, residual=residual, bnb=bnb, wimg=wimg, dy_amax=amax)
+            dx = ops.conv2d_dgrad(dc, w, N, H, W, cin, cout, k, k, s, p, residual=residual, bnb=bnb, wimg=wimg, dy_amax=amax,
+                                  accumulate=accumulate)
         else:
             assert residual is None and bnb is None
             dx = ops.gconv3x3_dgrad(dc, wexp, N, H, W, cin, s)
@@ -471,6 +472,22 @@
                     da1 = res
                     dc1 = _bn_bwd(blk.bn1, da1, r.c1, r.s1, rows_o, 2, dc_out=da1)
             first = blk.conv1
+            bnb = _tail_bnb(prev)
+            ds = blk.downsample
+            acc_ds = (ds is not None and bnb is None and ds[0].kernel_size[0] == 1 and ds[0].stride[0] == 2 and ds[0].padding[0] == 0
+                      and ds[0].groups == 1 and first.groups == 1 and ops.stream_mode() == 2)
+            if acc_ds:
+                dy = _conv_bwd(first, dc1, r.yin, N, Hi, Wi, None, None, side=side)
+                if pend is None:
+                    dcd = _bn_bwd(ds[1], dz, r.cd, r.sd, rows_o, 0, dc_out=dz)
+                else:
+                    dcd = _bn_bwd_part(ds[1], pend[0], pend[1], 2, dz, r.cd, r.sd, rows_o, dc_out=dz, dzmax=pend[2])
+                _conv_bwd(ds[0], dcd, r.yin, N, Hi, Wi, None, None, side=side, accumulate=dy)
+                pend = None
+                del dc1, da1, dz, dcd, r
+                if side is not None and side.hold:
+                    side.join()
+                continue
             if blk.downsample is not None:
                 if pend is None:
                     dcd = _bn_bwd(blk.downsample[1], dz, r.cd, r.sd, rows_o, 0, dc_out=dz)
@@ -479,7 +496,6 @@
                 resid = _conv_bwd(blk.downsample[0], dcd, r.yin, N, Hi, Wi, None, None, side=side)
             else:
                 resid = dz
-            bnb = _tail_bnb(prev)
             res = _conv_bwd(first, dc1, r.yin, N, Hi, Wi, None, None, residual=resid, side=side, bnb=bnb)
             if bnb is not None:
                 dy, part, mx = split(res)
diff --git a/oaprogressionmmf_amd/ops.py b/oaprogressionmmf_amd/ops.py
--- a/oaprogressionmmf_amd/ops.py
+++ b/oaprogressionmmf_amd/ops.py
@@ -152,8 +152,17 @@
     return lib().koaf_set_conv3x3_halo(int(mode))
 
 
-def set_stream(on):
-    return bool(lib().koaf_set_stream(1 if on else 0))
+_STREAM_MODE = {"0": 0, "1": 1}.get(os.environ.get("KOAF_STREAM", "2")[:1], 2)
+
+
+def set_stream(mode):
+    global _STREAM_MODE
+    _STREAM_MODE = max(0, min(2, int(mode)))
+    return int(lib().koaf_set_stream(_STREAM_MODE))
+
+
+def stream_mode():
+    return _STREAM_MODE
 
 
 def launch_log(on):
@@ -227,11 +236,17 @@
 
 
 def conv2d_dgrad(dy, w, N, H, W, Cin, Cout, KH, KW, stride, pad, residual=None, bnb=None, wimg=None, dy_amax=None,
-                 aplanes=None):
+                 aplanes=None, accumulate=None):
     L = lib()
     dyp, amp, app, like = _dy_args(dy, dy_amax)
     a16 = _a16(dy.c) if isinstance(dy, BnApply) else (_a16(bnb["c"]) if bnb is not None else 0)
-    dx = _empty((N, H, W, Cin), like)
+    if accumulate is not None:
+        if residual is not None or bnb is not None or tuple(accumulate.shape) != (N, H, W, Cin) or not accumulate.is_contiguous() \
+                or accumulate.dtype != torch.float32:
+            raise KoafError("conv2d_dgrad: accumulate takes a contiguous fp32 [N,H,W,Cin] tensor and excludes residual / bnb")
+        dx = accumulate
+    else:
+        dx = _empty((N, H, W, Cin), like)
     if aplanes is None:
         aplanes = ((APLANES_MASK & 2) and use_aplanes(wimg, KH, KW, Cout) and wimg[1] is not None and stride in (1, 2) and
                    (app is not None or dy_amax is not None))
@@ -244,13 +259,16 @@
     tag = f"conv_dgrad k{KH}s{stride} {Cin}->{Cout} px{N*H*W}"
     el = N * conv_out(H, KH, stride, pad) * conv_out(W, KW, stride, pad) * Cout + Cout * KH * KW * Cin + N * H * W * Cin
     el += N * H * W * Cin if residual is not None else 0
+    if accumulate is not None:
+        el = N * conv_out(H, 1, 2, 0) * conv_out(W, 1, 2, 0) * (Cout + 2 * Cin) + Cout * Cin
     mpp = 3 if (wimg is not None and (dy_amax is not None or app is not None)) else 6
     if app is not None:
         el += N * conv_out(H, KH, stride, pad) * conv_out(W, KW, stride, pad) * Cout
         tag += " apply"
     if bnb is None:
         check(L.koaf_conv2d_dgrad(dyp, _ptr(w), _ptr(dx), N, H, W, Cin, Cout, KH, KW, stride, pad,
-                                  _ptr(residual), _img(wimg), amp, app, dypp, a16, _stream()), "conv2d_dgrad")
+                                  _ptr(residual), _img(wimg), amp, app, dypp, a16, 1 if accumulate is not None else 0, _stream()),
+              "conv2d_dgrad")
         _prof_end(e0, "gemm", fl, tag, el, mpp=mpp)
         return dx
     sv, sv2 = bnb["saved"], bnb.get("saved2")
@@ -263,7 +281,7 @@
     rows = _i32(0)
     check(L.koaf_conv2d_dgrad_bnb(dyp, _ptr(w), _ptr(dx), N, H, W, Cin, Cout, KH, KW, stride, pad,
                                   _ptr(residual), ctypes.byref(kb), _ptr(part), ctypes.addressof(rows), _img(wimg),
-                                  amp, app, dypp, a16, _stream()), "conv2d_dgrad_bnb")
+                                  amp, app, dypp, a16, 0, _stream()), "conv2d_dgrad_bnb")
     el += N * H * W * Cin * (1 + (bnb.get("y") is not None) + (bnb.get("c2") is not None))
     _prof_end(e0, "gemm", fl, tag + " +bnb", el, mpp=mpp)
     if dzmax is not None:
```

New measurement: 4.118 knees/s, median of 6. About the same (+0.7%).
